# nanoporetech/bonito

Hardware: AMD Instinct MI355X
Metric: signal samples/sec/GPU (chunk=10000, batch=512) + read accuracy vs ref (higher is better)
Workload: dtype f16

## Files before the change

### bonito_amd/_lib.py

```python
import ctypes as C
import os

_HERE = os.path.dirname(os.path.abspath(__file__))
LIB_PATH = os.environ.get("BONITO_HIP_LIB") or os.path.join(_HERE, "libbonito_hip.so")


class HipEngineError(RuntimeError):
    """An entry point of libbonito_hip.so reported an error."""


class bh_layer_t(C.Structure):
    _fields_ = [
        ("kind", C.c_int32), ("in_size", C.c_int32), ("out_size", C.c_int32),
        ("winlen", C.c_int32), ("stride", C.c_int32), ("padding", C.c_int32),
        ("activation", C.c_int32), ("reverse", C.c_int32),
        ("nhead", C.c_int32), ("dim_ff", C.c_int32), ("win_left", C.c_int32), ("win_right", C.c_int32),
        ("scale_factor", C.c_int32), ("groups", C.c_int32), ("add_residual", C.c_int32), ("quantize", C.c_int32), ("reserved_i", C.c_int32 * 1),
        ("scale", C.c_float), ("clamp_lo", C.c_float), ("clamp_hi", C.c_float),
        ("blank_score", C.c_float), ("alpha", C.c_float), ("eps", C.c_float), ("reserved_f", C.c_float * 2),
        ("w0", C.c_void_p), ("b0", C.c_void_p), ("w1", C.c_void_p), ("b1", C.c_void_p),
        ("w2", C.c_void_p), ("w3", C.c_void_p), ("w4", C.c_void_p), ("w5", C.c_void_p),
    ]


BH_ACT = {None: 0, "none": 0, "swish": 1, "tanh": 2, "relu": 3}
BH_LAYER_CONV, BH_LAYER_LSTM, BH_LAYER_LINEAR_CRF, BH_LAYER_CLAMP = 1, 2, 3, 4
BH_LAYER_TRANSFORMER, BH_LAYER_UPSAMPLE, BH_LAYER_TCS_BLOCK, BH_LAYER_CTC_DECODER = 5, 6, 7, 8
BH_LAYER_DWCONV, BH_LAYER_RESIDUAL_PROJ, BH_LAYER_LINEAR = 9, 10, 11

_vp, _i, _f, _l, _sz = C.c_void_p, C.c_int, C.c_float, C.c_long, C.c_size_t

SIGNATURES = {
    "bh_last_error": (C.c_char_p, []),
    "bh_abi_version": (_i, []),
    "bh_sizeof_layer": (_sz, []),
    "bh_device_count": (_i, []),
    "bh_encoder_create": (_i, [C.POINTER(bh_layer_t), _i, _i, _i, _i, C.POINTER(_vp)]),
    "bh_encoder_destroy": (None, [_vp]),
    "bh_encoder_output_shape": (_i, [_vp, _i, C.POINTER(_i), C.POINTER(_i), C.POINTER(_i)]),
    "bh_encoder_forward": (_i, [_vp, _vp, _i, _i, _vp, _vp]),
    "bh_encoder_check": (_i, [_vp, _vp]),
    "bh_encoder_error_flag": (_i, [_vp]),
    "bh_encoder_last_ticket": (_l, [_vp]),
    "bh_encoder_error_flag_at": (_i, [_vp, _l]),
    "bh_encoder_ack": (_i, [_vp, _l]),
    "bh_encoder_describe": (_i, [_vp, C.c_char_p, _sz]),
    "bh_encoder_profile": (_i, [_vp, _i]),
    "bh_encoder_profile_read": (_i, [_vp, C.POINTER(C.c_float), C.POINTER(_i)]),
    "bh_crf_viterbi_workspace": (_sz, [_i, _i, _i]),
    "bh_crf_viterbi": (_i, [_vp, _i, _i, _i, _i, _f, _l, _l, _vp, _vp, _vp, _vp, _vp]),
    "bh_crf_reverse_complement": (_i, [_vp, _vp, _i, _i, _i, _i, _l, _l, _vp]),
    "bh_crf_logz": (_i, [_vp, _i, _i, _i, _f, _vp, _vp, _vp]),
    "bh_crf_seq_workspace": (_sz, [_i, _i, _i, _i]),
    "bh_crf_seq_logz": (_i, [_vp, _i, _i, _i, _i, _f, _l, _l, _vp, _i, _i, _vp, _vp, _vp, _vp]),
    "bh_crf_seq_viterbi": (_i, [_vp, _i, _i, _i, _i, _f, _l, _l, _vp, _i, _i, _vp, _vp, _vp, _vp, _vp]),
    "bh_crf_seq_logz_free": (_i, [_vp, _i, _i, _i, _f, _l, _l, _vp, _i, _i, _vp, _vp, _vp, _vp]),
    "bh_crf_logz_dense": (_i, [_vp, _i, _i, _i, _i, _f, _l, _l, _vp, _vp]),
    "bh_sw_workspace": (_sz, [_i, _i, _i]),
    "bh_sw_align": (_i, [_vp, _l, _vp, _vp, _l, _vp, _i, _i, _i, _i, _i, _vp, _sz, _vp, _vp, _l, _vp, _vp]),
    "bh_set_option": (_i, [C.c_char_p, _i]),
    "bh_signal_normalise": (_i, [_vp, _vp, _vp, _vp, _i, _i, C.c_double, C.c_double, C.c_double, C.c_double, C.c_double, C.c_double,
                            _i, _vp, _vp, _vp, _vp, _vp]),
    "bh_signal_chunks": (_i, [_vp, _vp, _vp, _vp, _vp, _vp, _vp, _vp, _vp, _vp, _i, _i, _vp, _vp]),
    "bh_crf_posterior_viterbi_workspace": (_sz, [_i, _i, _i]),
    "bh_crf_posterior_viterbi": (_i, [_vp, _i, _i, _i, _f, _vp, _vp, _vp, _vp]),
    "bh_beam_search_workspace": (_sz, [_i, _i, _i]),
    "bh_beam_search": (_i, [_vp, _i, _i, _i, _i, _f, _f, _f, _f, _vp, _vp, _vp, _vp, _vp, _vp]),
    "bh_linear": (_i, [_vp, _vp, _vp, _vp, _i, _i, _i, _i, _i, _i, _i, _f, _f, _f, _i, _i, _l, _l, _i, _vp]),
    "bh_linear_residual": (_i, [_vp, _vp, _vp, _vp, _i, _i, _i, _i, _i, _i, _i, _f, _f, _f, _i, _i, _l, _l, _i, _vp, _i, _f, _vp]),
    "bh_linear_qkv_rotary": (_i, [_vp, _vp, _vp, _vp, _i, _i, _i, _vp, _i, _f, _vp]),
    "bh_linear_last_kernel": (_i, []),
    "bh_conv1d_first": (_i, [_vp, _vp, _vp, _vp, _i, _i, _i, _i, _i, _i, _i, _f, _f, _l, _l, _vp]),
    "bh_conv1d_packed_halves": (_sz, [_i, _i, _i]),
    "bh_conv1d_pack": (_i, [_vp, _i, _i, _i, _vp]),
    "bh_conv1d": (_i, [_vp, _vp, _vp, _vp, _i, _i, _i, _i, _i, _i, _i, _i, _f, _f, _l, _l, _vp]),
    "bh_ctc_greedy_decode": (_i, [_vp, _vp, _i, _i, _f, _f, _vp, _vp, _vp, _vp, _vp]),
    "bh_ctc_beam_search_workspace": (_sz, [_l, _i, _i, _i]),
    "bh_ctc_beam_search": (_i, [_vp, _vp, _i, _i, _i, _f, _vp, _vp, _vp, _vp, _vp]),
    "bh_dwconv1d": (_i, [_vp, _vp, _vp, _i, _i, _i, _i, _i, _i, _vp]),
    "bh_rotary_table": (_i, [_i, _i, _vp]),
    "bh_attention": (_i, [_vp, _vp, _vp, _i, _i, _i, _i, _i, _i, _vp]),
    "bh_attention_prerotated": (_i, [_vp, _vp, _i, _i, _i, _i, _i, _i, _vp]),
    "bh_rmsnorm_residual": (_i, [_vp, _vp, _vp, _vp, _l, _i, _f, _f, _vp]),
    "bh_lstm_pack_whh": (_i, [_vp, _i, _vp]),
    "bh_host_compact": (_l, [_vp, _l, _vp]),
    "bh_host_chunk_rows": (_l, [_vp, _l, _i, _i, _l, _l, _vp]),
    "bh_host_format_read": (_l, [_vp, _vp, _vp, _vp, _i, _l, _l, _i, _i, _i, _i, _i, _i, C.c_double, C.c_char_p, C.c_char_p, _l, _l,
                                 _vp, _l, _vp, _vp]),
    "bh_host_mean_qscore": (C.c_double, [C.c_char_p, _l]),
    "bh_host_svb16_decode": (_l, [_vp, _l, _l, _vp]),
    "bh_lstm_workspace": (_sz, [_i, _i]),
    "bh_lstm_layer": (_i, [_vp, _vp, _vp, _i, _i, _i, _i, _vp, _vp, _i, _vp]),
    "bh_lstm_q8_layer": (_i, [_vp, _f, _vp, _vp, _vp, _i, _i, _i, _i, _i, _vp, _vp, _vp, _vp]),
    "bh_encoder_debug_read": (_i, [_vp, _vp, _sz, _sz]),
    "bh_encoder_set_option": (_i, [_vp, C.c_char_p, _i]),
}

_lib = None


def lib():
    global _lib
    if _lib is None:
        if not os.path.exists(LIB_PATH):
            raise HipEngineError(
                "%s not found: the MI355X engine is not built (run `python build.py`). "
                "bonito_amd has no CPU fallback." % LIB_PATH
            )
        import torch
        handle = C.CDLL(LIB_PATH)
        for name, (res, args) in SIGNATURES.items():
            fn = getattr(handle, name)
            fn.restype = res
            fn.argtypes = args
        if handle.bh_sizeof_layer() != C.sizeof(bh_layer_t):
            raise HipEngineError("bh_layer_t layout mismatch between include/bonito_hip.h and bonito_amd/_lib.py")
        _lib = handle
    return _lib


def last_error():
    msg = lib().bh_last_error()
    return msg.decode() if msg else ""


def check(rc, what=""):
    if rc != 0:
        raise HipEngineError("%s failed (rc=%d): %s" % (what or "libbonito_hip call", rc, last_error()))


def stream_ptr(device=None):
    import torch
    return C.c_void_p(torch.cuda.current_stream(device).cuda_stream)


def ptr(t):
    if t is None:
        return None
    return C.c_void_p(t.data_ptr())
```

### bonito_amd/csrc/abi.cpp

```cpp
#include <hip/hip_runtime.h>
#include <string.h>

#include <algorithm>
#include <cmath>
#include <vector>

#include "../../include/bonito_hip.h"
#include "common.h"
#include "devbuf.h"
#include "kernels.h"
#include "options.h"

extern "C" size_t bh_conv1d_packed_halves(int Cin, int Cout, int K) {
    size_t kp = ((size_t)K * Cin + 31) / 32 * 32;
    size_t c16 = ((size_t)Cout + 15) / 16 * 16;
    return kp * c16;
}
extern "C" int bh_conv1d_pack(const float* w, int Cin, int Cout, int K, uint16_t* packed) {
    BH_REQUIRE(w && packed && Cin > 0 && Cout > 0 && K > 0, "conv1d_pack: bad arguments");
    size_t kp = ((size_t)K * Cin + 31) / 32 * 32;
    size_t c16 = ((size_t)Cout + 15) / 16 * 16;
    memset(packed, 0, kp * c16 * 2);
    for (int f = 0; f < Cout; ++f)
        for (int c = 0; c < Cin; ++c)
// ... 25 lines not shown
                       row_s_hi, row_s_lo, row_lim, (hipStream_t)stream);
}
extern "C" int bh_linear_residual(const void* X, const void* W, const float* bias, void* out, int M, int N, int K, int ldx,
                                  int ldw, int ldo, int act, float scale, float clamp_lo, float clamp_hi, int gated,
                                  int row_div, long row_s_hi, long row_s_lo, int row_lim, const void* residual, int ldres,
                                  float res_scale, void* stream) {
    BH_REQUIRE(X && W && out && residual, "linear_residual: null pointer");
    return bh_k_linear(X, W, bias, out, M, N, K, ldx, ldw, ldo, act, scale, clamp_lo, clamp_hi, gated, row_div,
                       row_s_hi, row_s_lo, row_lim, (hipStream_t)stream, residual, ldres, res_scale);
}
extern "C" int bh_linear_qkv_rotary(const void* X, const void* W, const float* bias, void* out, int M, int D, int K,
                                    const float* cos_sin, int T, float qscale, void* stream) {
    BH_REQUIRE(X && W && out && cos_sin, "linear_qkv_rotary: null pointer");
    return bh_k_linear_qkv_rotary(X, W, bias, out, M, D, K, cos_sin, T, qscale, (hipStream_t)stream);
}
extern "C" int bh_linear_last_kernel(void) { return bh_k_linear_last_kernel(); }
extern "C" int bh_conv1d_first(const void* signal, const float* w, const float* bias, void* out, int N, int Lin,
                               int Cout, int K, int stride, int pad, int act, float clamp_lo, float clamp_hi,
                               long os_n, long os_t, void* stream) {
    BH_REQUIRE(signal && w && out && stride > 0, "conv1d_first: bad arguments");
    const int lout = conv_out_len(Lin, K, stride, pad);
    BH_REQUIRE(lout > 0, "conv1d_first: input too short");
    return bh_k_conv_first(signal, w, bias, out, N, Lin, lout, Cout, K, stride, pad, act, clamp_lo, clamp_hi, os_n,
                           os_t, (hipStream_t)stream);
}
extern "C" int bh_conv1d(const void* in, const void* wpacked, const float* bias, void* out, int N, int Lin, int Cin,
                         int Cout, int K, int stride, int pad, int act, float clamp_lo, float clamp_hi, long os_n,
                         long os_t, void* stream) {
    BH_REQUIRE(in && wpacked && out && stride > 0, "conv1d: bad arguments");
    const int lout = conv_out_len(Lin, K, stride, pad);
    BH_REQUIRE(lout > 0, "conv1d: input too short");
    return bh_k_conv_igemm(in, wpacked, bias, out, N, Lin, lout, Cin, Cout, K, stride, pad, act, clamp_lo, clamp_hi,
                           os_n, os_t, (hipStream_t)stream);
}
extern "C" int bh_rotary_table(int T, int dim, float* out) {
    BH_REQUIRE(out && T > 0 && dim > 0 && dim % 2 == 0, "rotary_table: bad arguments");
    const int half = dim / 2;
    for (int t = 0; t < T; ++t)
        for (int i = 0; i < half; ++i) {
            const float inv = 1.0f / powf(10000.0f, (float)(2 * i) / (float)dim);
            const float ang = (float)t * inv;
            out[((size_t)t * half + i) * 2] = cosf(ang);
            out[((size_t)t * half + i) * 2 + 1] = sinf(ang);
        }
    return 0;
}
extern "C" int bh_attention(const void* qkv, void* out, const float* cos_sin, int N, int T, int nhead, int head_dim,
                            int win_left, int win_right, void* stream) {
    BH_REQUIRE(qkv && out && cos_sin, "attention: null pointer");
    return bh_k_attention(qkv, out, cos_sin, N, T, nhead, head_dim, win_left, win_right, (hipStream_t)stream);
}
extern "C" int bh_attention_prerotated(const void* qkv, void* out, int N, int T, int nhead, int head_dim, int win_left, int win_right,
                                       void* stream) {
    BH_REQUIRE(qkv && out, "attention_prerotated: null pointer");
    return bh_k_attention_prerotated(qkv, out, N, T, nhead, head_dim, win_left, win_right, (hipStream_t)stream);
}
extern "C" int bh_rmsnorm_residual(const void* a, const void* x, const float* w, void* out, long M, int D, float alpha,
                                   float eps, void* stream) {
    BH_REQUIRE(a && x && w && out && M > 0, "rmsnorm_residual: bad arguments");
    return bh_k_rmsnorm_residual(a, x, w, out, M, D, alpha, eps, (hipStream_t)stream);
}
extern "C" int bh_ctc_greedy_decode(const float* logp, const long* offsets, int R, int classes, float qscale, float qbias,
                                    int8_t* labels, int8_t* qual, int* path, int* count, void* stream) {
    BH_REQUIRE(logp && offsets && labels && qual && path && count, "ctc_greedy_decode: null pointer");
    return bh_k_ctc_greedy(logp, offsets, R, classes, qscale, qbias, labels, qual, path, count, (hipStream_t)stream);
}
extern "C" size_t bh_ctc_beam_search_workspace(long total_steps, int R, int classes, int beam_size) {
    return bh_k_ctc_beam_workspace(total_steps, R, classes, beam_size);
}
extern "C" int bh_ctc_beam_search(const float* logp, const long* offsets, int R, int classes, int beam_size, float threshold,
                                  void* workspace, int8_t* labels, int* path, int* count, void* stream) {
    BH_REQUIRE(logp && offsets && workspace && labels && path && count, "ctc_beam_search: null pointer");
    return bh_k_ctc_prefix_beam(logp, offsets, R, classes, beam_size, threshold, workspace, labels, path, count,
                                (hipStream_t)stream);
}
extern "C" int bh_dwconv1d(const void* in, const float* w, void* out, int N, int Lin, int C, int K, int stride, int pad,
                           void* stream) {
    BH_REQUIRE(in && w && out && stride > 0, "dwconv1d: bad arguments");
    const int lout = conv_out_len(Lin, K, stride, pad);
    BH_REQUIRE(lout > 0, "dwconv1d: input too short");
    return bh_k_dwconv(in, w, out, N, Lin, lout, C, K, stride, pad, (hipStream_t)stream);
}
extern "C" size_t bh_lstm_workspace(int N, int H) { return bh_k_lstm_ws_bytes(N, H); }
extern "C" int bh_lstm_layer(const void* gates_in, const void* whh_packed, void* h_out, int T, int N, int H,
                             int reverse, void* workspace, int* err_flag, int flags, void* stream) {
    BH_REQUIRE(gates_in && whh_packed && h_out && err_flag && workspace, "lstm_layer: null pointer");
    BH_REQUIRE(T > 0, "lstm_layer: T must be positive");
    int rc = bh_k_fill_u16(h_out, 0xFFFFu, (size_t)T * N * H, (hipStream_t)stream);
    if (rc) return rc;
    if (H > 512 || (flags & 2)) {
        const int per = std::max(8, bh_k_lstm_geometry(BH_LSTM_STREAM, H).rings_per_launch(bh_cu_count()));
        for (int r0 = 0; r0 < N / 16; r0 += per) {
            const int nr = std::min(per, N / 16 - r0);
            rc = bh_k_lstm_layer_stream((const char*)gates_in + (size_t)r0 * 16 * 4 * H * 2, whh_packed,
                                        (char*)h_out + (size_t)r0 * 16 * H * 2, T, N, H, reverse, err_flag,
                                        (hipStream_t)stream, nr, (int*)workspace, flags & 1);
            if (rc) return rc;
        }
        return 0;
    }
    return bh_k_lstm_layer(gates_in, whh_packed, h_out, T, N, H, reverse, err_flag, (hipStream_t)stream, N / 16,
                           (int*)workspace, flags & 1);
}
extern "C" int bh_lstm_q8_layer(const void* x, float bound, const float* w_ih, const float* w_hh, const float* bias, int T, int N,
                                int H, int reverse, int variant, void* h16_out, int8_t* hq_frag, int32_t* sums, void* stream_) {
    BH_REQUIRE(x && w_ih && w_hh && h16_out && T > 0 && N > 0 && N % 16 == 0, "lstm_q8_layer: bad arguments");
    const int U = bh_k_lstm_q8_units(H, variant);
    BH_REQUIRE(U != 0, "lstm_q8_layer: hidden size %d is not covered by the 8-bit kernel", H);
    hipStream_t st = (hipStream_t)stream_;
    const int R = N / 16;
    const size_t tile = bh_k_lstm_q8_tile_bytes(H), wbytes = (size_t)4 * H * ((H + 63) / 64 * 64);
    std::vector<int8_t> pk(wbytes);
    std::vector<float> s_ih((size_t)4 * H), s_hh((size_t)4 * H), b((size_t)4 * H, 0.0f);
    DevBuf q_wih, q_whh, q_sx, q_sh, q_b, xq, ex, ws, err;
    if (bh_k_lstm_q8_pack(w_ih, H, U, pk.data(), s_ih.data()) || upload(q_wih, pk.data(), pk.size())) return -1;
    if (bh_k_lstm_q8_pack(w_hh, H, U, pk.data(), s_hh.data()) || upload(q_whh, pk.data(), pk.size())) return -1;
    const float xs = (float)((double)bound / 127.0);
    for (int j = 0; j < 4 * H; ++j) { s_ih[j] *= xs; s_hh[j] /= 127.0f; if (bias) b[j] = bias[j]; }
    if (upload_f32(q_sx, s_ih.data(), s_ih.size()) || upload_f32(q_sh, s_hh.data(), s_hh.size()) || upload_f32(q_b, b.data(), b.size())) return -1;
    if (xq.alloc((size_t)T * R * tile) || ex.alloc(4 * (size_t)R * tile) || ws.alloc(bh_k_lstm_ws_bytes(N, 1024)) || err.alloc(sizeof(int))) return -1;
    BH_CHECK_HIP(hipMemsetAsync(err.p, 0, sizeof(int), st));
    int rc = bh_k_quantise_rows(x, xq.p, T, N, H, R, bound, st);
    if (!rc) rc = bh_k_lstm_q8_arm(ex.p, R, H, st);
    if (rc) return rc;
    const int per = bh_k_lstm_q8_geometry(H, variant).rings_per_launch(bh_cu_count());
    BH_REQUIRE(per >= 1, "lstm_q8_layer: device has too few CUs for hidden size %d", H);
    for (int r0 = 0; r0 < R; r0 += per) {
        const int nr = std::min(per, R - r0);
        rc = bh_k_lstm_layer_q8((const char*)xq.p + (size_t)r0 * tile, q_wih.p, q_whh.p, (const float*)q_sx.p, (const float*)q_sh.p,
                                (const float*)q_b.p, hq_frag ? (char*)hq_frag + (size_t)r0 * tile : nullptr,
                                (char*)h16_out + (size_t)r0 * 16 * H * 2, (char*)ex.p + (size_t)r0 * tile, T, N, H, R, nr, reverse,
                                (int*)err.p, st, (int*)ws.p, 0, variant, sums ? sums + (size_t)r0 * 16 * 4 * H * 2 : nullptr,
                                (unsigned)bh::g_opt.lstm_max_spins);
        if (rc) return rc;
    }
    int flag = 0;
    BH_CHECK_HIP(hipMemcpyAsync(&flag, err.p, sizeof(int), hipMemcpyDeviceToHost, st));
    BH_CHECK_HIP(hipStreamSynchronize(st));
    BH_REQUIRE(flag == 0, "lstm_q8_layer: exchange timeout in the recurrent kernel");
    return 0;
}
extern "C" size_t bh_beam_search_workspace(int N, int T, int state_len) { return bh_k_beam_workspace(N, T, state_len); }
extern "C" int bh_beam_search(const void* scores, int N, int T, int state_len, int beam_width, float beam_cut,
                              float blank_score, float q_scale, float q_offset, void* workspace, int8_t* sequence,
                              int8_t* qstring, int8_t* moves, float* qfloat, void* stream) {
    BH_REQUIRE(scores && workspace && sequence && qstring && moves, "beam_search: null pointer");
    return bh_k_beam_search(scores, N, T, state_len, beam_width, beam_cut, blank_score, q_scale, q_offset, workspace,
                            sequence, qstring, moves, qfloat, (hipStream_t)stream);
}
extern "C" int bh_crf_reverse_complement(const void* in, void* out, int N, int T, int state_len, int layout_5s,
                                         long stride_n, long stride_t, void* stream) {
    BH_REQUIRE(in && out, "crf_reverse_complement: null pointer");
    return bh_k_crf_revcomp(in, out, N, T, state_len, layout_5s, stride_n, stride_t, (hipStream_t)stream);
}
extern "C" int bh_crf_logz(const void* scores, int N, int T, int state_len, float blank_score, void* workspace,
                           double* logz, void* stream) {
    BH_REQUIRE(scores && workspace && logz, "crf_logz: null pointer");
    return bh_k_crf_logz(scores, N, T, state_len, blank_score, workspace, logz, (hipStream_t)stream);
}
extern "C" size_t bh_crf_seq_workspace(int N, int T, int Lmax, int state_len) {
    return bh_k_crf_seq_workspace(N, T, Lmax, state_len);
}
extern "C" int bh_crf_seq_logz(const void* scores, int N, int T, int state_len, int layout_5s, float blank_score, long stride_n,
                               long stride_t, const void* targets, int Lmax, int target_bytes, const int32_t* target_lengths,
                               void* workspace, float* logz_out, void* stream) {
    BH_REQUIRE(scores && targets && target_lengths && workspace && logz_out, "crf_seq_logz: null pointer");
// ... 73 lines not shown
```

### bonito_amd/csrc/engine.cpp

```cpp
#include <hip/hip_runtime.h>
#include <stdarg.h>
#include <stdio.h>
#include <string.h>

#include <algorithm>
#include <atomic>
#include <cmath>
#include <string>
#include <vector>

#include "../../include/bonito_hip.h"
#include "common.h"
#include "devbuf.h"
#include "kernels.h"
#include "options.h"

static thread_local char g_err[1024] = "";
void bh_set_error(const char* fmt, ...) {
    va_list ap;
    va_start(ap, fmt);
    vsnprintf(g_err, sizeof(g_err), fmt, ap);
    va_end(ap);
}
extern "C" const char* bh_last_error(void) { return g_err; }
// ... 22 lines not shown
                    }
    return 0;
}

namespace {

struct Layer {
    bh_layer_t d;
    DevBuf w0, w1, w2, w3, w4, w5, b0, b1;
    bool fused_clamp = false;
    float clamp_lo = -INFINITY, clamp_hi = INFINITY;
    int cin_eff = 0, cout_eff = 0;
    bool pointwise = false;
    bool q8 = false;
    int q_variant = 0;
    float q_bound = 1.0f;
    DevBuf q_wih, q_whh, q_sx, q_sh;
};

enum Layout { L_SIGNAL, L_NLC, L_TNC };

struct ProfSpan {
    bh_encoder* e; hipStream_t st; int cls; hipEvent_t a = nullptr, b = nullptr;
    ProfSpan(bh_encoder* e_, hipStream_t st_, int cls_);
    ~ProfSpan();
};

static inline int pad8(int n) { return (n + 7) / 8 * 8; }

}

#include <mutex>
#include <unordered_map>
hipError_t bh_max_lds(const void* fn, int bytes) {
    static std::mutex mu;
    static std::unordered_map<unsigned long long, int> raised;
    int dev = 0;
    hipError_t e = hipGetDevice(&dev);
    if (e != hipSuccess) return e;
    const unsigned long long key = (unsigned long long)(uintptr_t)fn * 64ull + (unsigned)dev % 64u;
    {
        std::lock_guard<std::mutex> g(mu);
        auto it = raised.find(key);
        if (it != raised.end() && it->second >= bytes) return hipSuccess;
    }
    e = hipFuncSetAttribute(fn, hipFuncAttributeMaxDynamicSharedMemorySize, bytes);
    if (e == hipSuccess) {
        std::lock_guard<std::mutex> g(mu);
        int& have = raised[key];
        if (have < bytes) have = bytes;
    }
    return e;
}
int bh_cu_count() {
    static std::atomic<int> cached[64];
    int dev = 0, cus = 0;
    if (hipGetDevice(&dev) != hipSuccess || dev < 0 || dev >= 64) return 256;
    cus = cached[dev].load(std::memory_order_relaxed);
    if (cus > 0) return cus;
    if (hipDeviceGetAttribute(&cus, hipDeviceAttributeMultiprocessorCount, dev) != hipSuccess || cus <= 0) return 256;
    cached[dev].store(cus, std::memory_order_relaxed);
    return cus;
}

struct bh_encoder {
    int device = 0;
    int max_batch = 0, max_chunk = 0;
    int n_cus = 0;
    std::vector<Layer> layers;
    DevBuf act[3], gates, sig, err, lstm_ws;
    static constexpr int ERR_SLOTS = 64;
    int* err_host = nullptr;
    std::atomic<long> ticket{-1};
    std::atomic<long> checked{-1};
    std::atomic<int> sticky{0};
    int* cur_err = nullptr;
    int n_act = 2;
    hipStream_t fill_stream = nullptr;
    hipEvent_t fill_ready = nullptr, fill_done = nullptr;
    void* prefilled = nullptr;
    int lstm_prefill = 1;
    DevBuf q_act[2], q_ex;
    DevBuf ex16;
    int lstm_pair = 1;
    int norm_fuse = 0;
    int lstm_exchange = 1;
    int lstm_q8 = 1;
    DevBuf res;
    DevBuf t_qkv, t_mid, t_a, t_b, rot;
    int rot_len = 0;
    int out_features = 0;
    int lstm_force_slow = 0;
    int batch_pad = 16;
    int lstm_wide = 1;
    int attn_ring = 1;
    int lstm_fused = 3;
    bool profiling = false;
    struct Span { int cls; hipEvent_t a, b; };
    std::vector<Span> spans;
    ~bh_encoder() {
        for (auto& s : spans) { (void)hipEventDestroy(s.a); (void)hipEventDestroy(s.b); }
        if (fill_ready) (void)hipEventDestroy(fill_ready);
        if (fill_done) (void)hipEventDestroy(fill_done);
        if (fill_stream) (void)hipStreamDestroy(fill_stream);
        if (err_host) (void)hipHostFree(err_host);
    }
};

namespace {

ProfSpan::ProfSpan(bh_encoder* e_, hipStream_t st_, int cls_) : e(e_), st(st_), cls(cls_) {
    if (!e->profiling) return;
    if (hipEventCreate(&a) != hipSuccess || hipEventCreate(&b) != hipSuccess) { a = b = nullptr; return; }
    (void)hipEventRecord(a, st);
}
ProfSpan::~ProfSpan() {
    if (!a) return;
    (void)hipEventRecord(b, st);
    e->spans.push_back({cls, a, b});
}

struct Walk {
    int T = 0, C = 0;
    size_t act_bytes = 0, gate_bytes = 0;
    size_t qkv_bytes = 0, mid_bytes = 0, model_bytes = 0;
    int max_tokens = 0;
};
static int walk(const bh_encoder* e, int N, int L, Walk* w) {
    long len = L;
    int C = 1;
    size_t amax = 0;
    for (const auto& l : e->layers) {
        switch (l.d.kind) {
            case BH_LAYER_CONV:
                len = conv_out_len((int)len, l.d.winlen, l.d.stride, l.d.padding);
                BH_REQUIRE(len > 0, "encoder: chunk of %d samples is too short for the convolution stack", L);
                C = l.d.out_size;
                amax = std::max(amax, (size_t)N * len * std::max(l.cout_eff, C) * 2);
                break;
            case BH_LAYER_LSTM:
                C = l.d.out_size;
                amax = std::max(amax, (size_t)N * len * C * 2);
                w->gate_bytes = std::max(w->gate_bytes, (size_t)N * len * 4 * C * 2);
                break;
            case BH_LAYER_LINEAR_CRF:
                C = l.d.out_size;
                break;
            case BH_LAYER_LINEAR:
                C = l.d.out_size;
                amax = std::max(amax, (size_t)N * len * C * 2);
                break;
            case BH_LAYER_CLAMP:
                break;
            case BH_LAYER_TRANSFORMER: {
                const size_t M = (size_t)N * len;
                amax = std::max(amax, M * C * 2);
                w->qkv_bytes = std::max(w->qkv_bytes, M * 3 * l.d.in_size * 2);
                w->mid_bytes = std::max(w->mid_bytes, M * l.d.dim_ff * 2);
                w->model_bytes = std::max(w->model_bytes, M * l.d.in_size * 2);
                w->max_tokens = std::max(w->max_tokens, (int)len);
                break;
            }
            case BH_LAYER_DWCONV:
                len = conv_out_len((int)len, l.d.winlen, l.d.stride, l.d.padding);
                BH_REQUIRE(len > 0, "encoder: chunk of %d samples is too short for the convolution stack", L);
                amax = std::max(amax, (size_t)N * len * C * 2);
// ... 239 lines not shown
               "encoder_create: layer %zu: clamp must follow a convolution or linear layer", i);
    Layer& P = e->layers[i - 1];
    P.fused_clamp = true;
    P.clamp_lo = d.clamp_lo;
    P.clamp_hi = d.clamp_hi;
    cs.bound = std::max(fabsf(d.clamp_lo), fabsf(d.clamp_hi));
    return 0;
}

static int create_layer(bh_encoder* e, size_t i, const bh_layer_t& d, CreateState& cs) {
    Layer& L = e->layers[i];
    switch (d.kind) {
        case BH_LAYER_CONV: return create_conv(e, i, d, cs);
        case BH_LAYER_LSTM: return create_lstm(e, i, d, cs);
        case BH_LAYER_LINEAR_CRF:
            BH_REQUIRE(d.w0 && d.in_size > 0 && d.out_size > 0 && d.in_size % 8 == 0, "encoder_create: layer %zu: malformed linearcrfencoder", i);
            e->out_features = d.out_size;
            return create_linear(L, d, d.out_size);
        case BH_LAYER_LINEAR:
            BH_REQUIRE(d.w0 && d.in_size > 0 && d.out_size > 0 && d.in_size % 8 == 0 && d.out_size % 8 == 0 && cs.channels == d.in_size,
                       "encoder_create: layer %zu: linear needs in/out features %% 8 == 0 and %d input features (chain provides %d)", i,
                       d.in_size, cs.channels);
            cs.channels = cs.channels_eff = d.out_size;
            return create_linear(L, d, d.out_size);
        case BH_LAYER_TRANSFORMER: return create_transformer(e, i, d);
        case BH_LAYER_DWCONV:
            BH_REQUIRE(d.w0 && d.in_size > 0 && d.in_size % 8 == 0 && d.winlen > 0 && d.stride > 0 && cs.channels == d.in_size &&
                           cs.channels_eff == d.in_size,
                       "encoder_create: layer %zu: depthwise conv needs %d (multiple of 8) input channels, chain provides %d", i, d.in_size,
                       cs.channels);
            return upload_f32(L.w0, d.w0, (size_t)d.in_size * d.winlen);
        case BH_LAYER_RESIDUAL_PROJ:
            BH_REQUIRE(d.w0 && d.in_size % 8 == 0 && d.out_size % 8 == 0 && d.in_size > 0 && d.out_size > 0 && cs.channels == d.in_size &&
                           cs.channels_eff == d.in_size,
                       "encoder_create: layer %zu: residual projection shape mismatch", i);
            return create_with_bias(L, d, true);
        case BH_LAYER_CTC_DECODER:
            BH_REQUIRE(d.w0 && d.in_size % 8 == 0 && d.out_size >= 1 && d.out_size <= 8 && cs.channels == d.in_size,
                       "encoder_create: layer %zu: ctc decoder needs features %% 8 == 0 and <= 8 classes", i);
            e->out_features = d.out_size;
            return create_with_bias(L, d, false);
        case BH_LAYER_UPSAMPLE:
            BH_REQUIRE(d.w0 && d.in_size > 0 && d.scale_factor > 0 && d.in_size % 8 == 0, "encoder_create: layer %zu: malformed upsample", i);
            return create_linear(L, d, (size_t)d.scale_factor * d.in_size);
        case BH_LAYER_CLAMP: return create_clamp(e, i, d, cs);
        default: BH_REQUIRE(false, "encoder_create: layer %zu: kind %d is not supported by this build", i, d.kind);
    }
}

static int create_workspace(bh_encoder* e, const CreateState& cs) {
    const size_t n_layers = e->layers.size();
    const int last = e->layers[n_layers - 1].d.kind;
    BH_REQUIRE(last == BH_LAYER_LINEAR_CRF || last == BH_LAYER_CTC_DECODER ||
                   (n_layers >= 2 && last == BH_LAYER_CLAMP && e->layers[n_layers - 2].d.kind == BH_LAYER_LINEAR_CRF),
               "encoder_create: the chain must end in a linearcrfencoder (optionally followed by clamp) or a ctc decoder");
    const int Np = (e->max_batch + e->batch_pad - 1) / e->batch_pad * e->batch_pad;
    Walk w;
    if (walk(e, Np, e->max_chunk, &w)) return -2;
    const size_t ab = w.act_bytes;
    bool has_res = false;
    for (const auto& l : e->layers) has_res |= l.d.kind == BH_LAYER_RESIDUAL_PROJ;
    if (has_res && e->res.alloc(ab + 256)) return -1;
    for (size_t i = 0; i < n_layers; ++i)
        if (e->layers[i].d.kind == BH_LAYER_LSTM && next_kind(e, i) == BH_LAYER_LSTM) e->n_act = 3;
    if (e->n_act == 3) {
        if (e->act[2].alloc(ab + 256) || hipMemset(e->act[2].p, 0, e->act[2].bytes) != hipSuccess ||
            hipEventCreateWithFlags(&e->fill_ready, hipEventDisableTiming) != hipSuccess ||
            hipEventCreateWithFlags(&e->fill_done, hipEventDisableTiming) != hipSuccess) {
            bh_set_error("encoder_create: sentinel pre-fill resources");
            return -1;
        }
    }
    if (cs.any_q8) {
        if (e->q_act[0].alloc(ab + 256) || e->q_act[1].alloc(ab + 256) || e->q_ex.alloc((size_t)4 * (Np / 16) * 16 * 1024 + 256))
            return -1;
    }
    {
        size_t exb = 0;
        for (const auto& l : e->layers) {
            if (l.d.kind != BH_LAYER_LSTM) continue;
            if (lstm_may_share(l.d)) exb = std::max(exb, bh_k_lstm_wgx_ex_bytes(Np, l.d.out_size));
            if (lstm_may_wide(l.d)) exb = std::max(exb, bh_k_lstm_wide_ex_bytes(Np, l.d.out_size));
        }
        if (exb && e->ex16.alloc(exb + 256)) return -1;
    }
    if (e->act[0].alloc(ab + 256) || e->act[1].alloc(ab + 256) || e->gates.alloc(w.gate_bytes + 256) ||
        e->sig.alloc((size_t)Np * e->max_chunk * 2) || e->err.alloc(sizeof(int) * bh_encoder::ERR_SLOTS) ||
        e->lstm_ws.alloc(bh_k_lstm_ws_bytes(Np, 1024)))
        return -1;
    if (w.qkv_bytes) {
        if (e->t_qkv.alloc(w.qkv_bytes + 256) || e->t_mid.alloc(w.mid_bytes + 256) || e->t_a.alloc(w.model_bytes + 256) ||
            e->t_b.alloc(w.model_bytes + 256))
            return -1;
        std::vector<float> cs_table((size_t)w.max_tokens * 32 * 2);
        if (bh_rotary_table(w.max_tokens, 64, cs_table.data())) return -2;
        if (upload_f32(e->rot, cs_table.data(), cs_table.size())) return -1;
        e->rot_len = w.max_tokens;
    }
    if (hipHostMalloc((void**)&e->err_host, sizeof(int) * bh_encoder::ERR_SLOTS, hipHostMallocDefault) != hipSuccess) {
        bh_set_error("encoder_create: hipHostMalloc failed");
        return -1;
    }
    for (int i = 0; i < bh_encoder::ERR_SLOTS; ++i) e->err_host[i] = 0;
    e->cur_err = (int*)e->err.p;
    if (hipMemset(e->err.p, 0, sizeof(int) * bh_encoder::ERR_SLOTS) != hipSuccess || hipMemset(e->act[0].p, 0, e->act[0].bytes) != hipSuccess ||
        hipMemset(e->act[1].p, 0, e->act[1].bytes) != hipSuccess) {
        bh_set_error("encoder_create: hipMemset failed");
        return -1;
    }
    return 0;
}

}

extern "C" int bh_encoder_create(const bh_layer_t* layers, int n_layers, int device, int max_batch,
                                 int max_chunk, bh_encoder_t** out) {
    BH_REQUIRE(layers && n_layers > 0 && out, "encoder_create: bad arguments");
    BH_REQUIRE(max_batch > 0 && max_chunk > 0, "encoder_create: max_batch/max_chunk must be positive");
    int ndev = 0;
    BH_CHECK_HIP(hipGetDeviceCount(&ndev));
    BH_REQUIRE(ndev > 0, "encoder_create: no HIP device visible -- the MI355X engine has no CPU fallback");
    BH_REQUIRE(device >= 0 && device < ndev, "encoder_create: device %d out of range (%d visible)", device, ndev);
    int prev = 0;
    BH_CHECK_HIP(hipGetDevice(&prev));
    BH_CHECK_HIP(hipSetDevice(device));
    auto* e = new bh_encoder();
    e->device = device;
    e->max_batch = max_batch;
    e->max_chunk = max_chunk;
    auto fail = [&](int code) {
        delete e;
        (void)hipSetDevice(prev);
        return code;
    };
    if (hipDeviceGetAttribute(&e->n_cus, hipDeviceAttributeMultiprocessorCount, device) != hipSuccess) {
        bh_set_error("encoder_create: cannot query CU count");
        return fail(-1);
    }
    e->layers.resize(n_layers);
    for (int i = 0; i < n_layers; ++i) e->layers[i].d = layers[i];
    CreateState cs;
    for (int i = 0; i < n_layers; ++i) {
        if (int rc = create_layer(e, (size_t)i, layers[i], cs)) return fail(rc);
        bh_layer_t& d = e->layers[i].d;
        d.w0 = d.w1 = d.w2 = d.w3 = d.w4 = d.w5 = d.b0 = d.b1 = nullptr;
    }
    if (int rc = create_workspace(e, cs)) return fail(rc);
    (void)hipSetDevice(prev);
    *out = e;
    return 0;
}

extern "C" void bh_encoder_destroy(bh_encoder_t* enc) {
    if (!enc) return;
    int prev = 0;
    (void)hipGetDevice(&prev);
    (void)hipSetDevice(enc->device);
    delete enc;
    (void)hipSetDevice(prev);
}

extern "C" int bh_encoder_output_shape(const bh_encoder_t* enc, int L, int* T, int* C, int* stride) {
    BH_REQUIRE(enc && L > 0, "encoder_output_shape: bad arguments");
    Walk w;
    if (walk(enc, 16, L, &w)) return -2;
    if (T) *T = w.T;
    if (C) *C = w.C;
// ... 13 lines not shown
    const size_t ib = next_layer(e, i), ic = next_layer(e, ib);
    if (next_kind(e, i) != BH_LAYER_CONV || next_kind(e, ib) != BH_LAYER_CONV) return false;
    const Layer &a = e->layers[i], &b = e->layers[ib], &c = e->layers[ic];
    if (a.d.in_size != 1 || a.pointwise || b.pointwise || c.pointwise || b.d.add_residual || c.d.add_residual) return false;
    if (next_kind(e, ic) != BH_LAYER_LSTM) return false;
    if (!bh_k_conv_front3_ok(a.cout_eff, a.d.winlen, a.d.stride, b.cin_eff, b.cout_eff, b.d.winlen, b.d.stride, c.cin_eff, c.cout_eff,
                             c.d.winlen, c.d.stride))
        return false;
    if (a.d.out_size != b.d.in_size || b.d.out_size != c.d.in_size || c.cout_eff != c.d.out_size) return false;
    *j1 = ib;
    *j2 = ic;
    return true;
}
}

extern "C" int bh_encoder_describe(const bh_encoder_t* e, char* buf, size_t n) {
    BH_REQUIRE(e && buf && n > 0, "encoder_describe: bad arguments");
    std::string out;
    char line[256];
    int li = 0;
    for (const auto& l : e->layers) {
        const bh_layer_t& d = l.d;
        switch (d.kind) {
            case BH_LAYER_CONV: {
                size_t fj1 = 0, fj2 = 0;
                const bool front = d.in_size == 1 && conv_front3_at(e, (size_t)li, &fj1, &fj2);
                snprintf(line, sizeof(line), "%d conv %d->%d k%d s%d: %s\n", li, d.in_size, d.out_size, d.winlen, d.stride,
                         l.pointwise ? "gemm (pointwise)" : front ? "conv_front3_kernel (this and the next two convolutions in one kernel)"
                         : d.in_size == 1 ? "conv_first_kernel" : "conv_igemm_kernel / conv_ws_kernel");
                break;
            }
            case BH_LAYER_LSTM: {
                const LstmPlan p = lstm_plan(e, l, (e->max_batch + e->batch_pad - 1) / e->batch_pad * e->batch_pad);
                const int H = d.out_size, nks = H / 32, MT = bh_k_lstm_wg_units(H) / 4;
                char k[128];
                switch (p.family) {
                    case BH_LSTM_Q8: snprintf(k, sizeof(k), "lstm_layer_q8_kernel<%d,%d> (int8 W/x/h, i32 MFMA 16x16x64)", (H + 63) / 64, bh_k_lstm_q8_units(H, l.q_variant) / 4); break;
                    case BH_LSTM_CTA: snprintf(k, sizeof(k), "lstm_layer_cta_kernel<%d,%d>", nks, MT); break;
                    case BH_LSTM_WGX: snprintf(k, sizeof(k), "lstm_layer_%s_kernel<%d,%d>", p.pair_launch(p.n_rings) ? "wgx2" : "wgx", nks, MT); break;
                    case BH_LSTM_FUSED: snprintf(k, sizeof(k), "lstm_layer_fused_kernel<%d>", nks); break;
                    case BH_LSTM_WIDE: snprintf(k, sizeof(k), "gemm + lstm_layer_wide_kernel<%d,%s>", nks, p.handoff == HANDOFF_RING ? "true" : "false"); break;
                    case BH_LSTM_WAVE: snprintf(k, sizeof(k), "gemm + lstm_layer_kernel<%d,false>", nks); break;
                    default: snprintf(k, sizeof(k), "gemm + lstm_layer_kernel<%d,true> (weight streaming)", nks);
                }
                snprintf(line, sizeof(line), "%d lstm %d%s: %s\n", li, H, d.reverse ? " rev" : "", k);
                break;
            }
            case BH_LAYER_LINEAR_CRF: snprintf(line, sizeof(line), "%d linearcrfencoder %d->%d: gemm\n", li, d.in_size, d.out_size); break;
            case BH_LAYER_LINEAR: snprintf(line, sizeof(line), "%d linear %d->%d: gemm\n", li, d.in_size, d.out_size); break;
            case BH_LAYER_TRANSFORMER: {
                const bool ring = e->attn_ring && bh_k_attention_ring_serves(d.win_left, d.win_right);
                snprintf(line, sizeof(line), "%d transformer d%d h%d ff%d: gemm (Wqkv%s, out_proj, fc1 SwiGLU, fc2) + %s + rmsnorm_residual_kernel\n",
                         li, d.in_size, d.nhead, d.dim_ff, ring ? " + rotary" : "", ring ? "attention_ring_kernel" : "attention_kernel");
                break;
            }
            case BH_LAYER_UPSAMPLE: snprintf(line, sizeof(line), "%d linearupsample x%d: gemm\n", li, d.scale_factor); break;
            case BH_LAYER_CLAMP: snprintf(line, sizeof(line), "%d clamp: fused into the previous layer's epilogue\n", li); break;
            case BH_LAYER_DWCONV: snprintf(line, sizeof(line), "%d dwconv k%d: dwconv_kernel\n", li, d.winlen); break;
            case BH_LAYER_RESIDUAL_PROJ: snprintf(line, sizeof(line), "%d residual projection: gemm\n", li); break;
            case BH_LAYER_CTC_DECODER: snprintf(line, sizeof(line), "%d ctc decoder: ctc_head_kernel\n", li); break;
            default: snprintf(line, sizeof(line), "%d kind %d\n", li, d.kind);
        }
        out += line;
        ++li;
    }
    snprintf(buf, n, "%s", out.c_str());
    return 0;
}

namespace {

struct Cursor {
    const void* cur;
    Layout lay = L_SIGNAL;
    int len, C = 1;
    int which = 0;
    const void* cur_q = nullptr;
    int qi = 0;
    bool res_ready = false;
    int N, Np;
    hipStream_t st;
    void* scores;
    int n_act;
    void advance(void* dst) { cur = dst; which = (which + 1) % n_act; }
};

static int prefill_next(bh_encoder* e, const Cursor& c, size_t i, size_t rows) {
    if (e->n_act != 3 || !e->lstm_prefill || e->profiling) return 0;
    const size_t j = next_layer(e, i);
    if (j >= e->layers.size() || e->layers[j].d.kind != BH_LAYER_LSTM) return 0;
    const Layer& nx = e->layers[j];
    if (lstm_plan(e, nx, c.Np).handoff != HANDOFF_OUTPUT) return 0;
    if (!e->fill_stream) BH_CHECK_HIP(hipStreamCreateWithFlags(&e->fill_stream, hipStreamNonBlocking));
    void* spare = e->act[(c.which + 1) % 3].p;
    BH_CHECK_HIP(hipEventRecord(e->fill_ready, c.st));
    BH_CHECK_HIP(hipStreamWaitEvent(e->fill_stream, e->fill_ready, 0));
    const int rc = bh_k_fill_u16(spare, 0xFFFFu, rows * nx.d.out_size, e->fill_stream);
    if (rc) return rc;
    BH_CHECK_HIP(hipEventRecord(e->fill_done, e->fill_stream));
    e->prefilled = spare;
    return 0;
}

static int forward_conv(bh_encoder* e, size_t& i, Cursor& c) {
    const Layer& l = e->layers[i];
    const bh_layer_t& d = l.d;
    hipStream_t st = c.st;
    const int Np = c.Np, len = c.len;
    BH_REQUIRE(c.lay == L_SIGNAL || c.lay == L_NLC, "encoder_forward: convolution after a time-major layer");
    BH_REQUIRE(c.C == d.in_size, "encoder_forward: layer %zu expects %d channels, got %d", i, d.in_size, c.C);
    size_t fj1 = 0, fj2 = 0;
    if (c.lay == L_SIGNAL && conv_front3_at(e, i, &fj1, &fj2)) {
        const Layer &l2 = e->layers[fj1], &l3 = e->layers[fj2];
        const int len1 = conv_out_len(len, d.winlen, d.stride, d.padding);
        const int len2 = conv_out_len(len1, l2.d.winlen, l2.d.stride, l2.d.padding);
        const int len3 = conv_out_len(len2, l3.d.winlen, l3.d.stride, l3.d.padding);
        BH_REQUIRE(len1 > 0 && len2 > 0 && len3 > 0, "encoder_forward: chunk too short for the convolution stack");
        void* dst3 = e->act[c.which].p;
        int rc3 = prefill_next(e, c, fj2, (size_t)len3 * Np);
        if (rc3) return rc3;
        ProfSpan span(e, st, BH_PROF_CONV);
        rc3 = bh_k_conv_front3(c.cur, Np, len, (const float*)l.w0.p, (const float*)l.b0.p, d.winlen, d.padding, d.activation, l.clamp_lo,
                               l.clamp_hi, l2.w0.p, (const float*)l2.b0.p, l2.d.winlen, l2.d.padding, l2.d.activation, l2.clamp_lo,
                               l2.clamp_hi, l3.w0.p, (const float*)l3.b0.p, l3.cout_eff, l3.d.winlen, l3.d.stride, l3.d.padding,
                               l3.d.activation, l3.clamp_lo, l3.clamp_hi, dst3, (long)l3.cout_eff, (long)Np * l3.cout_eff, st);
        if (rc3) return rc3;
        c.advance(dst3); c.len = len3; c.C = l3.d.out_size; c.lay = L_TNC;
        i = fj2;
        return 0;
    }
    const int lout = conv_out_len(len, d.winlen, d.stride, d.padding);
    void* dst = e->act[c.which].p;
    const bool tnc = next_kind(e, i) == BH_LAYER_LSTM;
    const int co = l.cout_eff;
    const long os_n = tnc ? co : (long)lout * co;
    const long os_t = tnc ? (long)Np * co : co;
    int rc;
    if (tnc) { rc = prefill_next(e, c, i, (size_t)lout * Np); if (rc) return rc; }
    ProfSpan span(e, st, BH_PROF_CONV);
    if (l.pointwise && !tnc) {
        const void* rsd = d.add_residual ? e->res.p : nullptr;
        BH_REQUIRE(!d.add_residual || c.res_ready, "encoder_forward: layer %zu adds a residual that was never projected", i);
        rc = bh_k_linear(c.cur, l.w0.p, (const float*)l.b0.p, dst, Np * len, d.out_size, d.in_size, d.in_size,
                         d.in_size, d.out_size, d.activation, 1.0f, l.clamp_lo, l.clamp_hi, 0, 0, 0, 0, 0, st, rsd, d.out_size);
        if (d.add_residual) c.res_ready = false;
    } else if (c.lay == L_SIGNAL)
        rc = bh_k_conv_first(c.cur, (const float*)l.w0.p, (const float*)l.b0.p, dst, Np, len, lout,
                             co, d.winlen, d.stride, d.padding, d.activation, l.clamp_lo, l.clamp_hi, os_n, os_t, st);
    else
        rc = bh_k_conv_igemm(c.cur, l.w0.p, (const float*)l.b0.p, dst, Np, len, lout, l.cin_eff,
                             co, d.winlen, d.stride, d.padding, d.activation, l.clamp_lo, l.clamp_hi, os_n, os_t, st);
    if (rc) return rc;
    c.advance(dst); c.len = lout; c.C = d.out_size; c.lay = tnc ? L_TNC : L_NLC;
    return 0;
}

static int forward_lstm_q8(bh_encoder* e, size_t i, Cursor& c, const LstmPlan& p) {
    const Layer& l = e->layers[i];
    const bh_layer_t& d = l.d;
    hipStream_t st = c.st;
    const int H = d.out_size, len = c.len, Np = c.Np, R = p.n_rings;
    const size_t tile = bh_k_lstm_q8_tile_bytes(H);
    void* dst = e->act[c.which].p;
    const size_t j = next_layer(e, i);
    const bool next_q8 = j < e->layers.size() && e->layers[j].d.kind == BH_LAYER_LSTM && lstm_plan(e, e->layers[j], Np).family == BH_LSTM_Q8;
    int rc;
    const void* xq = c.cur_q;
    if (!xq) {
        ProfSpan span(e, st, BH_PROF_OTHER);
        rc = bh_k_quantise_rows(c.cur, e->q_act[c.qi].p, len, Np, H, R, l.q_bound, st);
        if (rc) return rc;
        xq = e->q_act[c.qi].p;
        c.qi ^= 1;
    }
    void* hq_out = next_q8 ? e->q_act[c.qi].p : nullptr;
    void* h16_out = next_q8 ? nullptr : dst;
    ProfSpan span(e, st, BH_PROF_LSTM_REC);
    rc = bh_k_lstm_q8_arm(e->q_ex.p, R, H, st);
    if (rc) return rc;
    for (int r0 = 0; r0 < R; r0 += p.rings_per_launch) {
        const int nr = std::min(p.rings_per_launch, R - r0);
        rc = bh_k_lstm_layer_q8((const char*)xq + (size_t)r0 * tile, l.q_wih.p, l.q_whh.p, (const float*)l.q_sx.p,
                                (const float*)l.q_sh.p, (const float*)l.b0.p,
                                hq_out ? (char*)hq_out + (size_t)r0 * tile : nullptr,
                                h16_out ? (char*)h16_out + (size_t)r0 * 16 * H * 2 : nullptr,
                                (char*)e->q_ex.p + (size_t)r0 * tile, len, Np, H, R, nr, d.reverse, e->cur_err, st,
                                (int*)e->lstm_ws.p, e->lstm_force_slow, l.q_variant, nullptr, (unsigned)bh::g_opt.lstm_max_spins);
        if (rc) return rc;
    }
    if (next_q8) { c.cur_q = hq_out; c.qi ^= 1; }
    else { c.cur_q = nullptr; c.advance(dst); }
    c.C = H;
    return 0;
}

static int forward_lstm(bh_encoder* e, size_t i, Cursor& c) {
    const Layer& l = e->layers[i];
    const bh_layer_t& d = l.d;
    hipStream_t st = c.st;
    BH_REQUIRE(c.lay == L_TNC, "encoder_forward: lstm needs time-major input");
    BH_REQUIRE(c.C == d.in_size, "encoder_forward: layer %zu expects %d features, got %d", i, d.in_size, c.C);
    const int H = d.out_size, len = c.len, Np = c.Np;
    const int M = len * Np;
    const LstmPlan p = lstm_plan(e, l, Np);
    BH_REQUIRE(p.rings_per_launch >= 1, "encoder_forward: device has too few CUs (%d) for hidden size %d", e->n_cus, H);
    if (p.family == BH_LSTM_Q8) return forward_lstm_q8(e, i, c, p);
    BH_REQUIRE(c.cur_q == nullptr, "encoder_forward: layer %zu would read int8 activations it cannot consume", i);
    int rc;
    void* dst = e->act[c.which].p;
    if (p.gate_w) {
        ProfSpan span(e, st, BH_PROF_LSTM_GEMM);
        rc = bh_k_linear(c.cur, p.gate_w, p.gate_b, e->gates.p, M, 4 * H, d.in_size, d.in_size, d.in_size, 4 * H, bh::ACT_NONE, 1.0f,
                         -INFINITY, INFINITY, 0, 0, 0, 0, 0, st);
        if (rc) return rc;
    }
    if (p.handoff == HANDOFF_OUTPUT) {
        if (e->prefilled == dst) {
            BH_CHECK_HIP(hipStreamWaitEvent(st, e->fill_done, 0));
        } else {
            ProfSpan span(e, st, BH_PROF_FILL);
            rc = bh_k_fill_u16(dst, 0xFFFFu, (size_t)M * H, st);
            if (rc) return rc;
        }
    }
    e->prefilled = nullptr;
    if (next_kind(e, i) == BH_LAYER_LSTM) { rc = prefill_next(e, c, i, (size_t)M); if (rc) return rc; }
    ProfSpan span(e, st, BH_PROF_LSTM_REC);
    const int n_rings = p.n_rings, rev = d.reverse, slow = e->lstm_force_slow;
    int* ws = (int*)e->lstm_ws.p;
    const float* bias = (const float*)l.b0.p;
    for (int r0 = 0; r0 < n_rings;) {
        const bool pair = p.pair_launch(n_rings - r0);
        const int nr = std::min(pair ? 2 * p.rings_per_launch : p.rings_per_launch, n_rings - r0);
        const size_t col = (size_t)r0 * p.geo.ring_chunks;
        const char* x = (const char*)c.cur + col * H * 2;
        const char* g = (const char*)e->gates.p + col * 4 * H * 2;
        char* h = (char*)dst + col * H * 2;
        char* ex = e->ex16.p ? (char*)e->ex16.p + (size_t)r0 * (p.geo.ring_chunks / 16) * (H / 32) * 1024 : nullptr;
        switch (pair ? BH_LSTM_WGX2 : p.family) {
            case BH_LSTM_WGX2:
                rc = bh_k_lstm_layer_wgx2(x, l.w4.p, bias, l.w3.p, h, ex, len, Np, H, n_rings, rev, e->cur_err, st, nr, ws, slow, r0 == 0);
                break;
            case BH_LSTM_WGX:
                rc = bh_k_lstm_layer_wgx(x, l.w4.p, bias, l.w3.p, h, ex, len, Np, H, n_rings, rev, e->cur_err, st, nr, ws, slow, r0 == 0);
                break;
            case BH_LSTM_WIDE:
                rc = bh_k_lstm_layer_wide(g, l.w3.p, h, len, Np, H, rev, e->cur_err, st, nr, ws, slow,
                                          p.handoff == HANDOFF_RING ? ex : nullptr, n_rings, r0 == 0);
                break;
            case BH_LSTM_CTA: rc = bh_k_lstm_layer_cta(x, l.w4.p, bias, l.w3.p, h, len, Np, H, rev, st, nr); break;
            case BH_LSTM_FUSED: rc = bh_k_lstm_layer_fused(x, l.w2.p, bias, l.w1.p, h, len, Np, H, rev, e->cur_err, st, nr, ws, slow); break;
            case BH_LSTM_WAVE: rc = bh_k_lstm_layer(g, l.w1.p, h, len, Np, H, rev, e->cur_err, st, nr, ws, slow); break;
            default: rc = bh_k_lstm_layer_stream(g, l.w1.p, h, len, Np, H, rev, e->cur_err, st, nr, ws, slow);
        }
        if (rc) return rc;
        r0 += nr;
    }
    c.advance(dst); c.C = H;
    return 0;
}

static int forward_linear_crf(bh_encoder* e, size_t i, Cursor& c) {
    const Layer& l = e->layers[i];
    const bh_layer_t& d = l.d;
    BH_REQUIRE(c.lay == L_TNC || c.lay == L_NLC, "encoder_forward: linearcrfencoder needs encoded input");
    BH_REQUIRE(c.C == d.in_size, "encoder_forward: layer %zu expects %d features, got %d", i, d.in_size, c.C);
    const float sc = d.scale != 0.0f ? d.scale : 1.0f;
    int rc;
    ProfSpan span(e, c.st, BH_PROF_CRF_LINEAR);
    if (c.lay == L_TNC)
        rc = bh_k_linear(c.cur, l.w0.p, (const float*)l.b0.p, c.scores, c.len * c.Np, d.out_size, d.in_size, d.in_size,
                         d.in_size, d.out_size, d.activation, sc, l.clamp_lo, l.clamp_hi, 0, c.Np, 1, c.len, c.N, c.st);
    else
        rc = bh_k_linear(c.cur, l.w0.p, (const float*)l.b0.p, c.scores, c.len * c.N, d.out_size, d.in_size, d.in_size,
                         d.in_size, d.out_size, d.activation, sc, l.clamp_lo, l.clamp_hi, 0, 0, 0, 0, 0, c.st);
    if (rc) return rc;
    c.C = d.out_size;
    return 0;
}

static int forward_linear(bh_encoder* e, size_t i, Cursor& c) {
    const Layer& l = e->layers[i];
    const bh_layer_t& d = l.d;
    BH_REQUIRE(c.lay == L_TNC || c.lay == L_NLC, "encoder_forward: linear needs encoded input");
    BH_REQUIRE(c.C == d.in_size, "encoder_forward: layer %zu expects %d features, got %d", i, d.in_size, c.C);
    void* dst = e->act[c.which].p;
    ProfSpan span(e, c.st, BH_PROF_OTHER);
    int rc = bh_k_linear(c.cur, l.w0.p, (const float*)l.b0.p, dst, c.len * c.Np, d.out_size, d.in_size, d.in_size, d.in_size,
                         d.out_size, bh::ACT_NONE, 1.0f, l.clamp_lo, l.clamp_hi, 0, 0, 0, 0, 0, c.st);
    if (rc) return rc;
    c.advance(dst); c.C = d.out_size;
    return 0;
}

static int forward_transformer(bh_encoder* e, size_t i, Cursor& c) {
    const Layer& l = e->layers[i];
    const bh_layer_t& d = l.d;
    hipStream_t st = c.st;
    const int len = c.len, N = c.N;
    BH_REQUIRE(c.lay == L_NLC, "encoder_forward: transformer layer needs [N][T][D] input");
    BH_REQUIRE(c.C == d.in_size, "encoder_forward: layer %zu expects d_model %d, got %d", i, d.in_size, c.C);
    BH_REQUIRE(len <= e->rot_len, "encoder_forward: %d tokens exceed the rotary table (%d)", len, e->rot_len);
    const int D = d.in_size, F = d.dim_ff;
    const int M = N * len;
    const float eps = d.eps > 0.0f ? d.eps : 1e-5f;
    int rc;
    const bool ring = e->attn_ring && bh_k_attention_ring_serves(d.win_left, d.win_right);
    const bool fuse = e->norm_fuse != 0;
    auto proj_norm = [&](const void* x, const void* w, const float* b, int K, const void* res, const float* gain, void* y) {
        int r = bh_k_linear(x, w, b, e->t_b.p, M, D, K, K, K, D, bh::ACT_NONE, 1.0f, -INFINITY, INFINITY, 0, 0, 0, 0, 0, st,
                            fuse ? res : nullptr, fuse ? D : 0, fuse ? d.alpha : 1.0f);
        if (!r) r = bh_k_rmsnorm_residual(e->t_b.p, fuse ? nullptr : res, gain, y, M, D, d.alpha, eps, st);
        return r;
    };
    {
        ProfSpan span(e, st, BH_PROF_ATTENTION);
        if (ring)
            rc = bh_k_linear_qkv_rotary(c.cur, l.w0.p, (const float*)l.b0.p, e->t_qkv.p, M, D, D, (const float*)e->rot.p,
                                        len, 0.125f * 1.4426950408889634f, st);
        else
            rc = bh_k_linear(c.cur, l.w0.p, (const float*)l.b0.p, e->t_qkv.p, M, 3 * D, D, D, D, 3 * D, bh::ACT_NONE,
                             1.0f, -INFINITY, INFINITY, 0, 0, 0, 0, 0, st);
        if (rc) return rc;
    }
    {
        ProfSpan span(e, st, BH_PROF_ATTENTION_CORE);
        if (ring)
            rc = bh_k_attention_prerotated(e->t_qkv.p, e->t_a.p, N, len, d.nhead, D / d.nhead, d.win_left, d.win_right, st);
        else
            rc = bh_k_attention(e->t_qkv.p, e->t_a.p, (const float*)e->rot.p, N, len, d.nhead, D / d.nhead,
                                d.win_left, d.win_right, st);
// ... 20 lines not shown
    return 0;
}

static int forward_dwconv(bh_encoder* e, size_t i, Cursor& c) {
    const Layer& l = e->layers[i];
    const bh_layer_t& d = l.d;
    BH_REQUIRE(c.lay == L_NLC && c.C == d.in_size, "encoder_forward: depthwise conv needs [N][L][%d] input", d.in_size);
    const int lout = conv_out_len(c.len, d.winlen, d.stride, d.padding);
    void* dst = e->act[c.which].p;
    ProfSpan span(e, c.st, BH_PROF_CONV);
    int rc = bh_k_dwconv(c.cur, (const float*)l.w0.p, dst, c.Np, c.len, lout, c.C, d.winlen, d.stride, d.padding, c.st);
    if (rc) return rc;
    c.advance(dst); c.len = lout;
    return 0;
}

static int forward_residual_proj(bh_encoder* e, size_t i, Cursor& c) {
    const Layer& l = e->layers[i];
    const bh_layer_t& d = l.d;
    BH_REQUIRE(c.lay == L_NLC && c.C == d.in_size, "encoder_forward: residual projection needs [N][L][%d] input", d.in_size);
    ProfSpan span(e, c.st, BH_PROF_CONV);
    int rc = bh_k_linear(c.cur, l.w0.p, (const float*)l.b0.p, e->res.p, c.Np * c.len, d.out_size, d.in_size, d.in_size,
                         d.in_size, d.out_size, bh::ACT_NONE, 1.0f, -INFINITY, INFINITY, 0, 0, 0, 0, 0, c.st);
    if (rc) return rc;
    c.res_ready = true;
    return 0;
}

static int forward_ctc_decoder(bh_encoder* e, size_t i, Cursor& c) {
    const Layer& l = e->layers[i];
    const bh_layer_t& d = l.d;
    BH_REQUIRE(c.lay == L_NLC && c.C == d.in_size, "encoder_forward: ctc decoder needs [N][T][%d] input", d.in_size);
    ProfSpan span(e, c.st, BH_PROF_CRF_LINEAR);
    int rc = bh_k_ctc_head(c.cur, (const float*)l.w0.p, (const float*)l.b0.p, c.scores, (long)c.N * c.len, d.in_size, d.out_size, c.st);
    if (rc) return rc;
    c.C = d.out_size;
    return 0;
}

static int forward_upsample(bh_encoder* e, size_t i, Cursor& c) {
    const Layer& l = e->layers[i];
    const bh_layer_t& d = l.d;
    BH_REQUIRE(c.lay == L_NLC && c.C == d.in_size, "encoder_forward: upsample needs [N][T][%d] input", d.in_size);
    const int D = d.in_size, sf = d.scale_factor;
    void* dst = e->act[c.which].p;
    ProfSpan span(e, c.st, BH_PROF_OTHER);
    int rc = bh_k_linear(c.cur, l.w0.p, (const float*)l.b0.p, dst, c.N * c.len, sf * D, D, D, D, sf * D, bh::ACT_NONE,
                         1.0f, -INFINITY, INFINITY, 0, 0, 0, 0, 0, c.st);
    if (rc) return rc;
    c.advance(dst); c.len *= sf;
    return 0;
}

}

extern "C" int bh_encoder_forward(bh_encoder_t* e, const void* signal, int N, int L, void* scores, void* stream_) {
    BH_REQUIRE(e && signal && scores, "encoder_forward: null argument");
    BH_REQUIRE(N > 0 && N <= e->max_batch, "encoder_forward: batch %d outside 1..%d", N, e->max_batch);
    BH_REQUIRE(L > 0 && L <= e->max_chunk, "encoder_forward: chunk %d outside 1..%d", L, e->max_chunk);
    hipStream_t st = (hipStream_t)stream_;
    int prev = 0;
    BH_CHECK_HIP(hipGetDevice(&prev));
    if (prev != e->device) BH_CHECK_HIP(hipSetDevice(e->device));
    struct Restore {
        int prev, dev;
        ~Restore() { if (prev != dev) (void)hipSetDevice(prev); }
    } restore{prev, e->device};

    {
        const long n = ++e->ticket;
        const int slot = (int)(n % bh_encoder::ERR_SLOTS);
        if (n - bh_encoder::ERR_SLOTS > e->checked.load()) e->sticky.fetch_or(((volatile int*)e->err_host)[slot]);
        ((volatile int*)e->err_host)[slot] = 0;
        e->cur_err = (int*)e->err.p + slot;
        BH_CHECK_HIP(hipMemsetAsync(e->cur_err, 0, sizeof(int), st));
    }
    const int Np = (N + e->batch_pad - 1) / e->batch_pad * e->batch_pad;
    if (Np != N) BH_CHECK_HIP(hipMemsetAsync((char*)e->sig.p + (size_t)N * L * 2, 0, (size_t)(Np - N) * L * 2, st));
    BH_CHECK_HIP(hipMemcpyAsync(e->sig.p, signal, (size_t)N * L * 2, hipMemcpyDeviceToDevice, st));

    e->prefilled = nullptr;
    Cursor c;
    c.cur = e->sig.p; c.len = L; c.N = N; c.Np = Np; c.st = st; c.scores = scores; c.n_act = e->n_act;
    for (size_t i = 0; i < e->layers.size(); ++i) {
        int rc = 0;
        switch (e->layers[i].d.kind) {
            case BH_LAYER_CLAMP: continue;
            case BH_LAYER_CONV: rc = forward_conv(e, i, c); break;
            case BH_LAYER_LSTM: rc = forward_lstm(e, i, c); break;
            case BH_LAYER_LINEAR_CRF: rc = forward_linear_crf(e, i, c); break;
            case BH_LAYER_LINEAR: rc = forward_linear(e, i, c); break;
            case BH_LAYER_TRANSFORMER: rc = forward_transformer(e, i, c); break;
            case BH_LAYER_DWCONV: rc = forward_dwconv(e, i, c); break;
            case BH_LAYER_RESIDUAL_PROJ: rc = forward_residual_proj(e, i, c); break;
            case BH_LAYER_CTC_DECODER: rc = forward_ctc_decoder(e, i, c); break;
            case BH_LAYER_UPSAMPLE: rc = forward_upsample(e, i, c); break;
            default: BH_REQUIRE(false, "encoder_forward: unsupported layer kind %d", e->layers[i].d.kind);
        }
        if (rc) return rc;
    }
    BH_CHECK_HIP(hipMemcpyAsync(e->err_host + (e->cur_err - (int*)e->err.p), e->cur_err, sizeof(int), hipMemcpyDeviceToHost, st));
    return 0;
}

extern "C" long bh_encoder_last_ticket(const bh_encoder_t* e) { return e ? e->ticket.load() : -1; }

extern "C" int bh_encoder_error_flag_at(const bh_encoder_t* e, long ticket) {
    if (!e || !e->err_host) return 0;
    const long cur = e->ticket.load();
    if (ticket < 0 || ticket > cur) return 0;
    if (cur - ticket >= bh_encoder::ERR_SLOTS) {
        bh_set_error("forward %ld is more than %d forwards old: its timeout flag has been recycled", ticket, bh_encoder::ERR_SLOTS);
        return -1;
    }
    const int flag = ((volatile const int*)e->err_host)[ticket % bh_encoder::ERR_SLOTS];
    if (flag) bh_set_error("device-side timeout in a persistent kernel (flag=%d, forward %ld): the scores of that forward are invalid", flag, ticket);
    return flag;
}

extern "C" int bh_encoder_ack(bh_encoder_t* e, long ticket) {
    BH_REQUIRE(e && e->err_host, "encoder_ack: null engine");
    const long cur = e->ticket.load();
    BH_REQUIRE(ticket >= 0 && ticket <= cur, "encoder_ack: forward %ld has not been issued (last %ld)", ticket, cur);
    if (cur - ticket >= bh_encoder::ERR_SLOTS) {
        bh_set_error("forward %ld is more than %d forwards old: its timeout flag has been recycled", ticket, bh_encoder::ERR_SLOTS);
        return -1;
    }
    ((volatile int*)e->err_host)[ticket % bh_encoder::ERR_SLOTS] = 0;
    return 0;
}

static int pending_flags(const bh_encoder_t* e) {
    int flag = e->sticky.load();
    const long cur = e->ticket.load();
    long lo = e->checked.load() + 1;
    if (lo < cur - bh_encoder::ERR_SLOTS + 1) lo = cur - bh_encoder::ERR_SLOTS + 1;
    if (lo < 0) lo = 0;
    for (long n = lo; n <= cur; ++n) flag |= ((volatile const int*)e->err_host)[n % bh_encoder::ERR_SLOTS];
    return flag;
}

extern "C" int bh_encoder_error_flag(const bh_encoder_t* e) {
    if (!e || !e->err_host) return 0;
    const int flag = pending_flags(e);
    if (flag) bh_set_error("device-side timeout in a persistent kernel (flag=%d): the scores of that forward are invalid", flag);
    return flag;
}

extern "C" int bh_encoder_check(bh_encoder_t* e, void* stream_) {
    BH_REQUIRE(e, "encoder_check: null engine");
    BH_CHECK_HIP(hipStreamSynchronize((hipStream_t)stream_));
    const int flag = pending_flags(e);
    e->sticky.store(0);
    if (flag) bh_set_error("device-side timeout in a persistent kernel (flag=%d)", flag);
    e->checked.store(e->ticket.load());
    return flag;
}

extern "C" int bh_encoder_profile(bh_encoder_t* e, int enable) {
    BH_REQUIRE(e, "encoder_profile: null engine");
    e->profiling = enable != 0;
    return 0;
}
extern "C" int bh_encoder_profile_read(bh_encoder_t* e, float* ms, int* launches) {
    BH_REQUIRE(e && ms && launches, "encoder_profile_read: null argument");
    for (int i = 0; i < BH_PROF_CLASSES; ++i) { ms[i] = 0.0f; launches[i] = 0; }
    for (auto& s : e->spans) {
        BH_CHECK_HIP(hipEventSynchronize(s.b));
        float t = 0.0f;
        BH_CHECK_HIP(hipEventElapsedTime(&t, s.a, s.b));
        if (s.cls >= 0 && s.cls < BH_PROF_CLASSES) { ms[s.cls] += t; launches[s.cls] += 1; }
        (void)hipEventDestroy(s.a); (void)hipEventDestroy(s.b);
    }
    e->spans.clear();
    return 0;
}

extern "C" int bh_encoder_debug_read(bh_encoder_t* e, void* host, size_t bytes, size_t offset) {
    BH_REQUIRE(e && host && offset + bytes <= e->lstm_ws.bytes, "encoder_debug_read: out of range");
    BH_CHECK_HIP(hipMemcpy(host, (char*)e->lstm_ws.p + offset, bytes, hipMemcpyDeviceToHost));
    return 0;
}
extern "C" int bh_encoder_set_option(bh_encoder_t* e, const char* name, int value) {
    BH_REQUIRE(e && name, "encoder_set_option: null argument");
    if (!strcmp(name, "lstm_force_slow")) { e->lstm_force_slow = (e->lstm_force_slow & ~1) | (value & 1); return 0; }
    if (!strcmp(name, "lstm_fused")) { e->lstm_fused = value; return 0; }
    if (!strcmp(name, "attn_ring")) { e->attn_ring = value; return 0; }
    if (!strcmp(name, "lstm_wide")) { e->lstm_wide = value; return 0; }
    if (!strcmp(name, "lstm_prefill")) { e->lstm_prefill = value; return 0; }
    if (!strcmp(name, "lstm_q8")) { e->lstm_q8 = value; return 0; }
    if (!strcmp(name, "lstm_exchange")) { e->lstm_exchange = value; return 0; }
    if (!strcmp(name, "lstm_pair")) { e->lstm_pair = value; return 0; }
    if (!strcmp(name, "norm_fuse")) { e->norm_fuse = value; return 0; }
    if (!strcmp(name, "gemm_v1")) { bh::g_opt.gemm_path = value; return 0; }
    if (!strcmp(name, "lstm_tune")) { e->lstm_force_slow = (e->lstm_force_slow & 1) | (value << 8); return 0; }
    BH_REQUIRE(false, "encoder_set_option: unknown option '%s'", name);
}
```

### bonito_amd/csrc/kernels.h

```cpp
#pragma once
#include <hip/hip_runtime.h>
#include <stdint.h>

int bh_k_linear(const void* X, const void* W, const float* bias, void* out, int M, int N, int K,
                int ldx, int ldw, int ldo, int act, float scale, float clamp_lo, float clamp_hi,
                int gated, int row_div, long row_s_hi, long row_s_lo, int row_lim, hipStream_t stream,
                const void* residual = nullptr, int ldres = 0, float res_scale = 1.0f);
int bh_k_linear_last_kernel();

int bh_k_conv_first(const void* signal, const float* w, const float* bias, void* out, int N, int Lin,
                    int Lout, int Cout, int K, int stride, int pad, int act, float clamp_lo,
                    float clamp_hi, long os_n, long os_t, hipStream_t stream);
int bh_k_conv_igemm(const void* in, const void* wpk, const float* bias, void* out, int N, int Lin,
                    int Lout, int Cin, int Cout, int K, int stride, int pad, int act, float clamp_lo,
                    float clamp_hi, long os_n, long os_t, hipStream_t stream);

enum bh_lstm_family { BH_LSTM_WAVE, BH_LSTM_FUSED, BH_LSTM_STREAM, BH_LSTM_WGX, BH_LSTM_WGX2, BH_LSTM_CTA, BH_LSTM_WIDE, BH_LSTM_Q8 };
struct bh_lstm_geometry {
    int ring_chunks = 16;
    int wgs_per_group = 0;
    int rings_per_slot = 1;
    int wgs_per_cu = 1;
    bool unlimited = false;
    int grid(int n_rings) const {
// ... 20 lines not shown
size_t bh_k_lstm_packed_bytes(int H);
int bh_k_lstm_wg_units(int H);
int bh_k_lstm_cta_units(int H);
int bh_k_lstm_layer_cta(const void* x, const void* wih_tiles, const float* bias, const void* whh_tiles, void* h_out, int T, int N,
                        int H, int reverse, hipStream_t stream, int n_rings);

int bh_k_crf_viterbi(const void* scores, int N, int T, int state_len, int layout_5s, float blank_score,
                     long s_n, long s_t, void* bp_ws, float* alpha_ws, int8_t* moves, int8_t* path,
                     float* best_score, hipStream_t stream);

int bh_k_crf_revcomp(const void* in, void* out, int N, int T, int state_len, int layout_5s, long s_n, long s_t,
                     hipStream_t stream);

size_t bh_k_crf_seq_workspace(int N, int T, int Lmax, int state_len);
int bh_k_crf_seq(const void* scores, int N, int T, int state_len, int layout_5s, float blank, long s_n, long s_t,
                 const void* targets, int target_bytes, int Lmax, const int* lens, void* workspace, float* out, int* align,
                 int mode, hipStream_t stream);
int bh_k_crf_logz_dense(const void* scores, int N, int T, int state_len, int layout_5s, float blank, long s_n, long s_t,
                        float* out, hipStream_t stream);

size_t bh_k_sw_workspace(int n, int max_seq, int max_ref);
int bh_k_sw_align(const void* seqs, long seq_stride, const int* seq_lens, const void* refs, long ref_stride, const int* ref_lens,
                  int n, int match, int mismatch, int gap_open, int gap_extend, void* workspace, size_t workspace_bytes,
                  int* result, unsigned* ops, long ops_stride, int* n_ops, hipStream_t stream);

size_t bh_k_beam_workspace(int N, int T, int state_len);
int bh_k_crf_logz(const void* scores, int N, int T, int state_len, float blank, void* workspace, double* logz_out,
                   hipStream_t stream);
int bh_k_beam_search(const void* scores, int N, int T, int state_len, int beam_width, float beam_cut,
                     float blank, float q_scale, float q_offset, void* workspace, int8_t* sequence,
                     int8_t* qstring, int8_t* moves, float* qfloat, hipStream_t stream);

int bh_k_attention(const void* qkv, void* out, const float* cos_sin, int N, int T, int nhead, int head_dim,
                   int win_left, int win_right, hipStream_t stream);
int bh_k_rmsnorm_residual(const void* a, const void* x, const float* w, void* out, long M, int D, float alpha,
                          float eps, hipStream_t stream);

int bh_k_dwconv(const void* in, const float* w, void* out, int N, int Lin, int Lout, int C, int K, int stride,
                int pad, hipStream_t stream);
int bh_k_ctc_head(const void* in, const float* w, const float* bias, void* out, long M, int features, int classes,
                  hipStream_t stream);
int bh_k_ctc_greedy(const float* logp, const long* offs, int R, int C, float qscale, float qbias, int8_t* seq,
                    int8_t* qual, int* path, int* count, hipStream_t stream);
size_t bh_k_ctc_beam_workspace(long total_steps, int R, int C, int beam_size);
int bh_k_ctc_prefix_beam(const float* logp, const long* offs, int R, int C, int beam_size, float threshold, void* workspace,
                         int8_t* labels, int* path, int* count, hipStream_t stream);
size_t bh_k_posterior_viterbi_workspace(int N, int T, int state_len);
int bh_k_posterior_viterbi(const void* scores, int N, int T, int state_len, float blank, void* workspace, int8_t* moves,
                           int8_t* path, hipStream_t stream);
int bh_k_conv_front3_ok(int c1_eff, int K1, int s1, int c2_in_eff, int c2_eff, int K2, int s2, int c3_in_eff, int c3_out, int K3, int s3);
int bh_k_conv_front3(const void* signal, int N, int L0, const float* w1, const float* b1, int K1, int pad1, int act1, float lo1, float hi1,
                     const void* w2pk, const float* b2, int K2, int pad2, int act2, float lo2, float hi2, const void* w3pk,
                     const float* b3, int Cout3, int K3, int stride3, int pad3, int act3, float lo3, float hi3, void* out, long os_n,
                     long os_t, hipStream_t stream);
int bh_k_linear_qkv_rotary(const void* X, const void* W, const float* bias, void* out, int M, int D, int K, const float* cos_sin,
                           int T, float qscale, hipStream_t stream);
int bh_k_attention_prerotated(const void* qkv, void* out, int N, int T, int nhead, int head_dim, int win_left, int win_right,
                              hipStream_t stream);
inline bool bh_k_attention_ring_serves(int win_left, int win_right) {
    return win_left >= 0 && win_right >= 0 && win_left <= 128 && win_right <= 144;
}
int bh_k_signal_normalise(const int16_t* raw, const long* offs, const float* cal_scale, const float* cal_offset, int R,
                          int strategy, double qa, double qb, double shift_mult, double scale_mult, double fixed_shift,
                          double fixed_scale, int do_trim, double* shift, double* scale, int* weak, int* trim, hipStream_t stream);
int bh_k_signal_chunks(const int16_t* raw, const long* offs, const float* cal_scale, const float* cal_offset, const double* shift,
                       const double* scale, const int* weak, const int* chunk_read, const long* chunk_start, const long* chunk_len,
                       int n_chunks, int L, void* out, hipStream_t stream);
int bh_k_lstm_wide_ok(int H);
int bh_k_lstm_layer_wide(const void* gates_perm, const void* whh_tiles, void* h_out, int T, int N, int H, int reverse,
                         int* err_flag, hipStream_t stream, int n_rings, int* xcc_ws, int force_slow, void* ex = nullptr, int R = 0,
                         int arm = 0);
size_t bh_k_lstm_wide_ex_bytes(int N, int H);

int bh_k_lstm_q8_units(int H, int variant);
bh_lstm_geometry bh_k_lstm_q8_geometry(int H, int variant);
size_t bh_k_lstm_q8_tile_bytes(int H);
int bh_k_lstm_q8_pack(const float* w, int H, int U, int8_t* packed, float* scale);
int bh_k_quantise_rows(const void* x, void* out, int T, int N, int H, int R, float bound, hipStream_t stream);
int bh_k_lstm_q8_arm(void* ex, int R, int H, hipStream_t stream);
int bh_k_lstm_layer_q8(const void* xq, const void* wih, const void* whh, const float* sx, const float* sh, const float* bias,
                       void* hq_out, void* h16_out, void* ex, int T, int N, int H, int R, int n_rings, int reverse, int* err_flag,
                       hipStream_t stream, int* xcc_ws, int flags, int variant, int* dbg, unsigned max_spins);
size_t bh_k_lstm_wgx_ex_bytes(int N, int H);
int bh_k_lstm_layer_wgx(const void* x, const void* wih_tiles, const float* bias, const void* whh_tiles, void* h_out, void* ex, int T,
                        int N, int H, int R, int reverse, int* err_flag, hipStream_t stream, int n_rings, int* xcc_ws, int force_slow,
                        int arm);
int bh_k_lstm_layer_wgx2(const void* x, const void* wih_tiles, const float* bias, const void* whh_tiles, void* h_out, void* ex, int T,
                        int N, int H, int R, int reverse, int* err_flag, hipStream_t stream, int n_rings, int* xcc_ws, int force_slow,
                        int arm);
```

### bonito_amd/csrc/lstm.hip

```cpp
#include <string.h>
#include <type_traits>

#include "common.h"
#include "kernels.h"
#include "options.h"

namespace bh {

struct LstmArgs {
    const half_t* G;
    const half_t* whh;
    half_t* h;
    int T, N, H;
    int n_rings;
    int reverse;
    int* err;
    unsigned max_spins;
    int* xcc_ws;
    int force_slow;
    int tune;
};

__device__ __forceinline__ int xcc_id() {
    return (int)(__builtin_amdgcn_s_getreg(20 | (0 << 6) | (3 << 11)) & 0xF);
}

__device__ __forceinline__ bool ring_store_policy(const LstmArgs& p, int ring, int slice, int nsl, int lane) {
    int* slot = p.xcc_ws + (long)ring * nsl;
    const int mine = xcc_id();
    if (lane == 0) __hip_atomic_store(slot + slice, mine, __ATOMIC_RELAXED, __HIP_MEMORY_SCOPE_AGENT);
    unsigned spins = 0;
    bool ok = false;
    while (true) {
        bool any_unset = false, any_other = false;
        for (int i = lane; i < nsl; i += 64) {
            const int v = __hip_atomic_load(slot + i, __ATOMIC_RELAXED, __HIP_MEMORY_SCOPE_AGENT);
            any_unset |= v < 0;
            any_other |= v != mine;
        }
        if (!__any(any_unset)) { ok = !__any(any_other); break; }
        if (++spins > p.max_spins) break;
        __builtin_amdgcn_s_sleep(4);
    }
    return ok && !p.force_slow;
}

constexpr unsigned SENTINEL_MASK = 0x40004000u;

typedef unsigned short __attribute__((may_alias)) u16_alias_t;
typedef unsigned long long __attribute__((may_alias)) u64_alias_t;

__device__ __forceinline__ float tanh_gate(float x) { return __builtin_fmaf(-2.0f, rcpf_(__expf(2.0f * x) + 1.0f), 1.0f); }

__device__ __forceinline__ float lstm_cell(float ai, float af, float ag, float ao, float& c) {
    const float ei = __expf(-__builtin_amdgcn_fmed3f(ai, -25.0f, 25.0f));
    const float ef = __expf(-__builtin_amdgcn_fmed3f(af, -25.0f, 25.0f));
    const float eg = __expf(-2.0f * __builtin_amdgcn_fmed3f(ag, -12.5f, 12.5f));
    const float eo = __expf(-__builtin_amdgcn_fmed3f(ao, -25.0f, 25.0f));
    const float didg = __fmul_rn(1.0f + ei, 1.0f + eg);
    const float df = 1.0f + ef;
    const float num = __builtin_fmaf(c, didg, __fmul_rn(1.0f - eg, df));
    c = __fmul_rn(num, rcpf_(__fmul_rn(df, didg)));
    const float ec = __expf(-2.0f * __builtin_amdgcn_fmed3f(c, -12.5f, 12.5f));
    const float hv = __fmul_rn(1.0f - ec, rcpf_(__fmul_rn(1.0f + ec, 1.0f + eo)));
    return (fabsf(hv) <= 1.0f) ? hv : 0.0f;
}

template <int NKS, bool STREAM>
__global__ __launch_bounds__(256, 1) void lstm_layer_kernel(LstmArgs p) {
    const int lane = threadIdx.x & 63;
    const int wave = __builtin_amdgcn_readfirstlane(threadIdx.x >> 6);
    constexpr int H = NKS * 32;
    constexpr int NSL = H / 16;
    const int xcd = blockIdx.x & 7;
    const int lwg = blockIdx.x >> 3;
    constexpr int WPR = NSL / 4;
    const int rg = STREAM ? lwg / WPR : lwg / NSL;
    const int slice = STREAM ? (lwg - rg * WPR) * 4 + wave : lwg - rg * NSL;
    const int ring = STREAM ? rg * 8 + xcd : (rg * 4 + wave) * 8 + xcd;
    if (ring >= p.n_rings) return;
    const half_t* wbase = p.whh + ((long)slice * 4 * NKS * 64 + lane) * 8;

    half8_t w[STREAM ? 1 : 4][STREAM ? 1 : NKS];
// ... 248 lines not shown
        }
        half4_t ho;
#pragma unroll
        for (int i = 0; i < 4; ++i) {
            const float hv = lstm_cell(acc[0][i], acc[1][i], acc[2][i], acc[3][i], cst[i]);
            ho[i] = (half_t)hv;
        }
#pragma unroll
        for (int ks = 0; ks < NKS; ++ks) asm volatile("" : "+v"(xf[ks]));
        unsigned long long packed = __builtin_bit_cast(unsigned long long, ho);
        unsigned long long* dst = (unsigned long long*)(p.h + ((long)t * p.N + n) * H + hu0);
        if (fast) *dst = packed;
        else __hip_atomic_store(dst, packed, __ATOMIC_RELAXED, __HIP_MEMORY_SCOPE_AGENT);
        if (p.tune & 4) st_rec += __builtin_readcyclecounter() - pc3;
    }
    if ((p.tune & 4) && lane == 0) {
        long long* st = (long long*)((char*)p.xcc_ws + (((size_t)p.n_rings * NSL * sizeof(int) + 64 + 7) & ~(size_t)7)) + ((long)ring * NSL + slice) * 8;
        st[0] = __builtin_readcyclecounter() - st_t0;
        st[1] = st_poll;
        st[2] = st_rounds;
        st[3] = st_first_ok;
        st[4] = st_x;
        st[5] = st_re;
        st[6] = st_rec;
        st[7] = st_hist;
    }
}

__device__ __forceinline__ void mfma16_av(const half8_t& a_agpr, const half8_t& b, float4_t& c) {
    asm("v_mfma_f32_16x16x32_f16 %0, %1, %2, %0" : "+v"(c) : "a"(a_agpr), "v"(b));
}
__device__ __forceinline__ void mfma16_vv(const half8_t& a, const half8_t& b, float4_t& c) {
    asm("v_mfma_f32_16x16x32_f16 %0, %1, %2, %0" : "+v"(c) : "v"(a), "v"(b));
}
template <int MT>
__device__ __forceinline__ void mfma_settle_v(float4_t (&c)[MT]) {
    if constexpr (MT == 3) asm volatile("s_nop 15\n\ts_nop 7" : "+v"(c[0]), "+v"(c[1]), "+v"(c[2]));
    else asm volatile("s_nop 15\n\ts_nop 7" : "+v"(c[0]), "+v"(c[1]), "+v"(c[2]), "+v"(c[3]));
}

__device__ __forceinline__ unsigned lds_addr(const char* p) { return (unsigned)(size_t)(__attribute__((address_space(3))) const char*)p; }
#include "ringstep3_mfma.inc"
#include "ringstep3p_mfma.inc"
template <int NKS, int MT>
__device__ __forceinline__ void ring_stream(float4_t (&xacc)[MT], float (&cst)[MT], float (&hv)[MT], const half8_t (&whh)[MT][NKS],
                                            const half8_t (&wih)[MT][NKS], const float4_t (&bias)[MT], unsigned hb, unsigned xb) {
    if constexpr (NKS == 12 && MT == 3) ringstep3_mfma(xacc, cst, hv, whh, wih, bias, hb, xb);
}
template <int NKS, int MT, int KQ>
__device__ __forceinline__ void ring_stream_paired(float4_t (&xacc)[MT], float (&cst)[MT], float (&hv)[MT], const half8_t (&whh)[MT][NKS],
                                                   const half8_t (&wih)[MT][NKS], const float4_t (&bias)[MT], unsigned hb, unsigned xb,
                                                   unsigned long long& bad, unsigned pm0, const char* exo, const unsigned (&vp)[KQ],
                                                   unsigned xm0, const char* xsrc, unsigned vx, unsigned hbo, unsigned sga, unsigned rda,
                                                   unsigned vmy, unsigned vh, const char* exs, const char* exa, const char* hrow, unsigned fast) {
    if constexpr (NKS == 12 && MT == 3)
        ringstep3p_mfma(xacc, cst, hv, whh, wih, bias, hb, xb, bad, pm0, exo, vp, xm0, xsrc, vx, hbo, sga, rda, vmy, vh, exs, exa, hrow, fast);
}
#include "ringstep3u_mfma.inc"
template <int NKS, int MT, int KQ, int HOFF, int XOFF, int VOFF, int PMO, int XMO>
__device__ __forceinline__ void ring_stream_unrolled(float4_t (&xacc)[MT], float (&cst)[MT], float (&hv)[MT], const half8_t (&whh)[MT][NKS],
                                                     const half8_t (&wih)[MT][NKS], const float4_t (&bias)[MT], unsigned hb, unsigned xb,
                                                     unsigned long long& bad, unsigned pm0, const char* exo, const unsigned (&vp)[KQ],
                                                     unsigned xm0, const char* xsrc, unsigned vx, unsigned hbo, unsigned sga, unsigned rda,
                                                     unsigned vmy, unsigned vh, const char* exs, const char* exa, const char* hrow, unsigned fast) {
    if constexpr (NKS == 12 && MT == 3)
        ringstep3u_mfma<HOFF, XOFF, VOFF, PMO, XMO>(xacc, cst, hv, whh, wih, bias, hb, xb, bad, pm0, exo, vp, xm0, xsrc, vx, hbo, sga, rda, vmy, vh, exs,
                                                    exa, hrow, fast);
}
#include "ringstep3r_mfma.inc"
template <int NKS, int MT>
__device__ __forceinline__ void ring_stream_rec(float4_t (&xacc)[MT], float (&cst)[MT], float (&hv)[MT], const half8_t (&whh)[MT][NKS],
                                                const half8_t (&wih)[MT][NKS], const float4_t (&bias)[MT], unsigned hb) {
    if constexpr (NKS == 12 && MT == 3) ringstep3r_mfma(xacc, cst, hv, whh, wih, bias, hb, 0u);
}
__device__ __forceinline__ void dma16_wgx(const char* g, char* lds) {
    const unsigned l = (unsigned)__builtin_amdgcn_readfirstlane((int)(unsigned)(size_t)(__attribute__((address_space(3))) char*)lds);
    asm volatile("s_mov_b32 m0, %0\n\ts_nop 0\n\tglobal_load_lds_dwordx4 %1, off" ::"s"(l), "v"(g) : "memory");
}

struct LstmWgxArgs {
    LstmFusedArgs f;
    char* ex;
    int R;
};

template <int IMM, bool POLL>
__device__ __forceinline__ void dma16_s(const char* sbase, unsigned voff, unsigned lds_a) {
    if constexpr (POLL)
        asm volatile("s_mov_b32 m0, %0\n\ts_nop 0\n\tglobal_load_lds_dwordx4 %1, %2 offset:%3 sc0 sc1" ::"s"(lds_a), "v"(voff), "s"(sbase), "i"(IMM) : "memory");
    else
        asm volatile("s_mov_b32 m0, %0\n\ts_nop 0\n\tglobal_load_lds_dwordx4 %1, %2 offset:%3" ::"s"(lds_a), "v"(voff), "s"(sbase), "i"(IMM) : "memory");
}
template <bool SC1>
__device__ __forceinline__ void store8_s(const char* sbase, unsigned voff, unsigned long long v) {
    if constexpr (SC1) asm volatile("global_store_dwordx2 %0, %1, %2 sc1" ::"v"(voff), "v"(v), "s"(sbase) : "memory");
    else asm volatile("global_store_dwordx2 %0, %1, %2" ::"v"(voff), "v"(v), "s"(sbase) : "memory");
}

template <int NKS, int MT>
__global__ __launch_bounds__(256, 1) void lstm_layer_wgx_kernel(LstmWgxArgs wp) {
    extern __shared__ __attribute__((aligned(16))) char smem[];
    const LstmFusedArgs& fp = wp.f;
    const LstmArgs& p = fp.a;
    constexpr int H = NKS * 32, U = 4 * MT, NSL = H / U, WPR = NSL / 4, KQ = (NKS + 3) / 4, TILE = NKS * 1024;
    constexpr bool EXACT = NKS % 4 == 0;
    static_assert(H % (4 * U) == 0, "four slices per workgroup");
    const int lane = threadIdx.x & 63;
    const int wave = __builtin_amdgcn_readfirstlane(threadIdx.x >> 6);
    const int xcd = blockIdx.x & 7;
    const int lwg = blockIdx.x >> 3;
    const int rl = lwg / WPR;
    const int ring = rl * 8 + ((p.tune & 32) ? ((xcd + (lwg - rl * WPR)) & 7) : xcd);
    const int slice = (lwg - rl * WPR) * 4 + wave;
    if (ring >= p.n_rings) return;

    char* hbuf = smem;
    char* xbuf = smem + 2 * TILE;
    char* stage = smem + 5 * TILE + wave * (16 * U * 2);

    half8_t whh[MT][NKS], wih[MT][NKS];
#pragma unroll
    for (int m = 0; m < MT; ++m)
#pragma unroll
        for (int ks = 0; ks < NKS; ++ks) {
            const long o = ((((long)slice * MT + m) * NKS + ks) * 64 + lane) * 8;
            whh[m][ks] = *(const half8_t*)(p.whh + o);
            wih[m][ks] = *(const half8_t*)(fp.wih + o);
        }
    const int c = lane & 15, q = lane >> 4;
    float cst[MT];
    float4_t bias4[MT];
#pragma unroll
    for (int m = 0; m < MT; ++m) {
        cst[m] = 0.f;
#pragma unroll
        for (int i = 0; i < 4; ++i) bias4[m][i] = fp.bias[i * H + slice * U + q * MT + m];
    }
    bool dead = false;
    const bool fast = ring_store_policy(p, ring, slice, NSL, lane);

    int t = p.reverse ? p.T - 1 : 0;
    const int dt = p.reverse ? -1 : 1;
    const half_t* xptr = fp.x + ((long)(ring * 16 + c) * H + q * 8);
    const long x_row = (long)p.N * H;
    const int lo = lane * 16;
    const long slot_stride = (long)wp.R * TILE;
    char* exr = wp.ex + (long)ring * TILE;

    constexpr int PARTS = U / 4;
    const bool mover = lane < 16 * PARTS;
    const int cc = lane / PARTS, part = lane - cc * PARTS;
    const int u0 = slice * U + part * 4;
    const int my_byte = (((u0 >> 5) * 64 + ((u0 >> 3) & 3) * 16 + cc) << 4) + (u0 & 7) * 2;

    uint4_t hq[KQ];
    float4_t xacc[MT];
    auto x_phase = [&](const char* xb) {
#pragma unroll
        for (int m = 0; m < MT; ++m) xacc[m] = bias4[m];
        half8_t b_cur = *(const half8_t*)(xb + lo), b_nxt = b_cur;
#pragma unroll
        for (int ks = 0; ks < NKS; ++ks) {
            if (ks + 1 < NKS) b_nxt = *(const half8_t*)(xb + (ks + 1) * 1024 + lo);
#pragma unroll
            for (int m = 0; m < MT; ++m) {
                if (m < MT - 1) mfma16_av(wih[m][ks], b_cur, xacc[m]);
                else mfma16_vv(wih[m][ks], b_cur, xacc[m]);
// ... 122 lines not shown
            u16_alias_t* sg = (u16_alias_t*)stage + c * U + q * MT;
#pragma unroll
            for (int m = 0; m < MT; ++m) sg[m] = __builtin_bit_cast(unsigned short, ho[m]);
            if (mover) {
                const unsigned long long packed = *(const u64_alias_t*)((half_t*)stage + cc * U + part * 4);
                if constexpr (STREAM) {
                    const char* exs = exr + (long)(step & 3) * slot_stride;
                    if (fast) store8_s<false>(exs, (unsigned)my_byte, packed); else store8_s<true>(exs, (unsigned)my_byte, packed);
                    if (step >= 2 && step + 2 < p.T) {
                        const char* exa = exr + (long)((step + 2) & 3) * slot_stride;
                        if (fast) store8_s<false>(exa, (unsigned)my_byte, ~0ull); else store8_s<true>(exa, (unsigned)my_byte, ~0ull);
                    }
                    store8_s<false>((const char*)p.h + (long)t * row_bytes, vh_off, packed);
                } else {
                unsigned long long* dst = (unsigned long long*)(exr + (long)(step & 3) * slot_stride + my_byte);
                if (fast) *dst = packed;
                else __hip_atomic_store(dst, packed, __ATOMIC_RELAXED, __HIP_MEMORY_SCOPE_AGENT);
                if (step >= 2 && step + 2 < p.T) {
                    unsigned long long* ra = (unsigned long long*)(exr + (long)((step + 2) & 3) * slot_stride + my_byte);
                    if (fast) *ra = ~0ull;
                    else __hip_atomic_store(ra, ~0ull, __ATOMIC_RELAXED, __HIP_MEMORY_SCOPE_AGENT);
                }
                *(unsigned long long*)(p.h + ((long)t * p.N + ring * 16 + cc) * H + slice * U + part * 4) = packed;
                }
            }
        }
        if (step + 1 < p.T) {
            const char* src = exr + (long)(step & 3) * slot_stride;
            __amdgpu_buffer_rsrc_t rs = __builtin_amdgcn_make_buffer_rsrc((void*)src, 0, TILE, 0x00020000);
#pragma unroll
            for (int kk = 0; kk < KQ; ++kk) {
                const int ks = wave + 4 * kk;
                if (EXACT || ks < NKS) hq[kk] = __builtin_amdgcn_raw_buffer_load_b128(rs, ks * 1024 + lo, 0, (int)0x80000010);
            }
        }
        const long long pc3 = (p.tune & 4) ? __builtin_readcyclecounter() : 0;
        x_phase(xbuf + ((step + 1) % 3) * TILE);
        if (p.tune & 4) {
            const long long now = __builtin_readcyclecounter();
            st_bar += pc2 - pc1; st_rec += pc3 - pc2; st_x += now - pc3;
            st_mf += pcm - pc2; st_gate += pcg - pcm; st_store += pc3 - pcg;
        }
    }
    if ((p.tune & 4) && lane == 0) {
        long long* st = (long long*)((char*)p.xcc_ws + (((size_t)p.n_rings * NSL * sizeof(int) + 64 + 7) & ~(size_t)7)) + ((long)ring * NSL + slice) * 16;
        st[0] = __builtin_readcyclecounter() - st_t0;
        st[1] = st_poll; st[2] = st_rounds; st[3] = st_first_ok; st[4] = st_x; st[5] = st_bar; st[6] = st_rec; st[7] = st_hist;
        st[8] = 0; st[9] = 0; st[10] = st_mf; st[11] = st_gate; st[12] = st_store;
        st[13] = (long long)__builtin_amdgcn_s_memrealtime() - st_r0;
    }
}

__device__ __forceinline__ void dma16_poll(const char* g, char* lds) {
    const unsigned l = (unsigned)__builtin_amdgcn_readfirstlane((int)(unsigned)(size_t)(__attribute__((address_space(3))) char*)lds);
    asm volatile("s_mov_b32 m0, %0\n\ts_nop 0\n\tglobal_load_lds_dwordx4 %1, off sc0 sc1" ::"s"(l), "v"(g) : "memory");
}
__device__ __forceinline__ void wait_vm(int n) {
    switch (n) {
        case 0: __builtin_amdgcn_s_waitcnt(0x0F70); break;
        case 1: __builtin_amdgcn_s_waitcnt(0x0F71); break;
        case 2: __builtin_amdgcn_s_waitcnt(0x0F72); break;
        case 3: __builtin_amdgcn_s_waitcnt(0x0F73); break;
        case 4: __builtin_amdgcn_s_waitcnt(0x0F74); break;
        case 5: __builtin_amdgcn_s_waitcnt(0x0F75); break;
        case 6: __builtin_amdgcn_s_waitcnt(0x0F76); break;
        case 7: __builtin_amdgcn_s_waitcnt(0x0F77); break;
        case 8: __builtin_amdgcn_s_waitcnt(0x0F78); break;
        case 9: __builtin_amdgcn_s_waitcnt(0x0F79); break;
        case 10: __builtin_amdgcn_s_waitcnt(0x0F7A); break;
        case 11: __builtin_amdgcn_s_waitcnt(0x0F7B); break;
        default: __builtin_amdgcn_s_waitcnt(0x0F7C); break;
    }
    asm volatile("" ::: "memory");
}

template <int NKS, int MT, bool STATS = false>
__global__ __launch_bounds__(256, 1) void lstm_layer_wgx2_kernel(LstmWgxArgs wp) {
    extern __shared__ __attribute__((aligned(16))) char smem[];
    const LstmFusedArgs& fp = wp.f;
    const LstmArgs& p = fp.a;
    constexpr int H = NKS * 32, U = 4 * MT, NSL = H / U, WPR = NSL / 4, KQ = (NKS + 3) / 4, TILE = NKS * 1024;
    constexpr bool EXACT = NKS % 4 == 0;
    static_assert(H % (4 * U) == 0, "four slices per workgroup");
    const int lane = threadIdx.x & 63;
    const int wave = __builtin_amdgcn_readfirstlane(threadIdx.x >> 6);
    const int xcd = blockIdx.x & 7;
    const int lwg = blockIdx.x >> 3;
    const int rl = lwg / WPR;
    const int n_pairs = (p.n_rings + 1) >> 1;
    const int pair = rl * 8 + ((p.tune & 32) ? ((xcd + (lwg - rl * WPR)) & 7) : xcd);
    const int slice = (lwg - rl * WPR) * 4 + wave;
    if (pair >= n_pairs) return;
    const int ring_of[2] = {pair, pair + n_pairs};
    const bool two = ring_of[1] < p.n_rings;

    char* hbuf = smem;
    char* xbuf = smem + 4 * TILE;
    char* stage = smem + 8 * TILE + wave * (16 * U * 2);

    half8_t whh[MT][NKS], wih[MT][NKS];
#pragma unroll
    for (int m = 0; m < MT; ++m)
#pragma unroll
        for (int ks = 0; ks < NKS; ++ks) {
            const long o = ((((long)slice * MT + m) * NKS + ks) * 64 + lane) * 8;
            whh[m][ks] = *(const half8_t*)(p.whh + o);
            wih[m][ks] = *(const half8_t*)(fp.wih + o);
        }
    const int c = lane & 15, q = lane >> 4;
    float4_t bias4[MT];
#pragma unroll
    for (int m = 0; m < MT; ++m)
#pragma unroll
        for (int i = 0; i < 4; ++i) bias4[m][i] = fp.bias[i * H + slice * U + q * MT + m];
    bool dead = false;
    const int dt = p.reverse ? -1 : 1;
    const int t0 = p.reverse ? p.T - 1 : 0;
    const long x_row = (long)p.N * H;
    const int lo = lane * 16;
    const long slot_stride = (long)wp.R * TILE;
    constexpr int PARTS = U / 4;
    const int ml = lane < 16 * PARTS ? lane : lane - 16 * PARTS;
    const int cc = ml / PARTS, part = ml - cc * PARTS;
    const int u0 = slice * U + part * 4;
    const int my_byte = (((u0 >> 5) * 64 + ((u0 >> 3) & 3) * 16 + cc) << 4) + (u0 & 7) * 2;
    int n_poll = 0, n_dma = 0;
#pragma unroll
    for (int kk = 0; kk < KQ; ++kk) {
        n_poll += (EXACT || wave + 4 * kk < NKS) ? 1 : 0;
        n_dma += (EXACT || (3 - wave) + 4 * kk < NKS) ? 1 : 0;
    }

    float cst[2][MT];
    float4_t xacc[2][MT];
    bool fast[2];
    const half_t* xptr[2];
    char* exr[2];
    int since[2] = {0, 0};
#pragma unroll
    for (int r = 0; r < 2; ++r) {
        const int ring = (r == 0 || two) ? ring_of[r] : ring_of[0];
        fast[r] = (r == 0 || two) ? ring_store_policy(p, ring, slice, NSL, lane) : false;
        xptr[r] = fp.x + ((long)(ring * 16 + c) * H + q * 8);
        exr[r] = wp.ex + (long)ring * TILE;
#pragma unroll
        for (int m = 0; m < MT; ++m) cst[r][m] = 0.f;
    }

    constexpr bool FASTPATH = NKS == 12 && MT == 3;
    const unsigned smem_a = lds_addr(smem);
    unsigned vx_off[2], vh_off[2], vp_off[KQ];
#pragma unroll
    for (int r = 0; r < 2; ++r) {
        const int ring = (r == 0 || two) ? ring_of[r] : ring_of[0];
        vx_off[r] = (unsigned)(((ring * 16 + c) * H + q * 8) * 2 + (3 - wave) * 64);
        vh_off[r] = (unsigned)(((ring * 16 + cc) * H + slice * U + part * 4) * 2);
    }
#pragma unroll
    for (int kk = 0; kk < KQ; ++kk) vp_off[kk] = (unsigned)(lo + (wave + 4 * kk) * 1024);
    const unsigned stage_a = lds_addr(stage);
    unsigned fast_u[2];
#pragma unroll
    for (int r = 0; r < 2; ++r)
        asm("s_cmp_lg_u64 %1, 0\n\ts_cselect_b32 %0, 1, 0" : "=s"(fast_u[r]) : "s"(__builtin_amdgcn_ballot_w64(fast[r])) : "scc");
    const long row_bytes = x_row * 2;
    const char* xrow2 = (const char*)fp.x + (long)(p.T > 2 ? t0 + 2 * dt : t0) * row_bytes;
    const char* xrow_any = (const char*)fp.x + (long)t0 * row_bytes;
    char* hrow = (char*)p.h + (long)t0 * row_bytes;

    auto x_phase = [&](const char* xb, float4_t (&xa)[MT]) {
#pragma unroll
        for (int m = 0; m < MT; ++m) xa[m] = bias4[m];
        half8_t b_cur = *(const half8_t*)(xb + lo), b_nxt = b_cur;
#pragma unroll
        for (int ks = 0; ks < NKS; ++ks) {
            if (ks + 1 < NKS) b_nxt = *(const half8_t*)(xb + (ks + 1) * 1024 + lo);
#pragma unroll
            for (int m = 0; m < MT; ++m) {
                if (m < MT - 1) mfma16_av(wih[m][ks], b_cur, xa[m]);
                else mfma16_vv(wih[m][ks], b_cur, xa[m]);
            }
            b_cur = b_nxt;
        }
        mfma_settle_v<MT>(xa);
    };
    auto x_dma = [&](const half_t* xp, char* xb, int tt, int slot) {
#pragma unroll
        for (int kk = 0; kk < KQ; ++kk) {
            const int ks = (3 - wave) + 4 * kk;
            if (EXACT || ks < NKS) dma16_wgx((const char*)(xp + (long)tt * x_row + ks * 32), xb + (slot * NKS + ks) * 1024);
        }
    };
    auto poll_dma = [&](const char* exbase, int slot, char* hb, unsigned mask) {
        const char* src = exbase + (long)slot * slot_stride + lo;
#pragma unroll
        for (int kk = 0; kk < KQ; ++kk) {
            const int ks = wave + 4 * kk;
            if ((EXACT || ks < NKS) && (mask & (1u << kk))) dma16_poll(src + ks * 1024, hb + ks * 1024);
        }
    };

#pragma unroll
    for (int r = 0; r < 2; ++r)
        if (r == 0 || two) {
            x_dma(xptr[r], xbuf + r * 2 * TILE, t0, 0);
            x_dma(xptr[r], xbuf + r * 2 * TILE, p.T > 1 ? t0 + dt : t0, 1);
        }
    if constexpr (NKS == 12 && MT == 3) {
#pragma unroll
        for (int r = 0; r < 2; ++r)
#pragma unroll
            for (int kk = 0; kk < KQ; ++kk)
                *(uint4_t*)(hbuf + r * 2 * TILE + (wave + 4 * kk) * 1024 + lo) = uint4_t{0u, 0u, 0u, 0u};
    }
    wait_vm(0);
    __syncthreads();
#pragma unroll
    for (int r = 0; r < 2; ++r)
        if (r == 0 || two) x_phase(xbuf + r * 2 * TILE, xacc[r]);

    long long st_poll = 0, st_bar = 0, st_slow = 0, st_sec[6] = {0, 0, 0, 0, 0, 0};
    const long long st_t0 = __builtin_readcyclecounter();
    const long long st_r0 = (p.tune & 4) ? (long long)__builtin_amdgcn_s_memrealtime() : 0;

    auto check_begin = [&](int rr, int st, uint4_t (&chk)[KQ]) {
        wait_vm(since[rr]);
        const char* hb = hbuf + (rr * 2 + (st & 1)) * TILE;
#pragma unroll
        for (int kk = 0; kk < KQ; ++kk) {
            const int ks = wave + 4 * kk;
            if (EXACT || ks < NKS) chk[kk] = *(const uint4_t*)(hb + ks * 1024 + lo);
        }
    };
    auto check_end = [&](int rr, int st, uint4_t (&chk)[KQ]) {
        char* hb = hbuf + (rr * 2 + (st & 1)) * TILE;
        unsigned spins = dead ? p.max_spins : 0u;
        while (true) {
            unsigned pend = 0;
#pragma unroll
            for (int kk = 0; kk < KQ; ++kk) {
                const int ks = wave + 4 * kk;
                if ((EXACT || ks < NKS) && __any(((chk[kk].x | chk[kk].y | chk[kk].z | chk[kk].w) & SENTINEL_MASK) != 0)) pend |= (1u << kk);
            }
            if (pend == 0) break;
            if (++spins > p.max_spins) {
                if (lane == 0 && !dead) atomicExch(p.err, 1);
                dead = true;
                break;
            }
            if (!(p.tune & 1)) __builtin_amdgcn_s_sleep(1);
            poll_dma(exr[rr], (st - 1) & 3, hb, pend);
            wait_vm(0);
#pragma unroll
            for (int kk = 0; kk < KQ; ++kk) {
                const int ks = wave + 4 * kk;
                if (EXACT || ks < NKS) chk[kk] = *(const uint4_t*)(hb + ks * 1024 + lo);
            }
        }
    };

    auto ring_step = [&](auto rc, auto two_c, int step, int t) {
        constexpr int r = decltype(rc)::value;
        constexpr bool TWO = decltype(two_c)::value;
        if constexpr (FASTPATH && TWO) {
            constexpr int o = r ^ 1;
            const int par = step & 1;
            const long long q0 = STATS ? __builtin_readcyclecounter() : 0;
            __syncthreads();
            const long long q1 = STATS ? __builtin_readcyclecounter() : 0;
            const int step_o = r == 0 ? step : step + 1;
            const bool chk_o = step_o >= 1 && step_o < p.T;
            const char* exo = exr[o] + (long)((step_o - 1) & 3) * slot_stride;
            const unsigned pm0 = (unsigned)__builtin_amdgcn_readfirstlane((int)(smem_a + (o * 2 + ((step_o & 1) ^ (chk_o ? 0 : 1))) * TILE + wave * 1024));
            const unsigned hbo = smem_a + (o * 2 + (step_o & 1)) * TILE + wave * 1024 + lo;
            const char* xsrc = (step + 2 < p.T) ? xrow2 : xrow_any;
            const unsigned xm0 = (unsigned)__builtin_amdgcn_readfirstlane((int)(smem_a + (4 + r * 2 + par) * TILE + (3 - wave) * 1024));
            unsigned long long bad;
            float hv[MT];
            const char* exs = exr[r] + (long)(step & 3) * slot_stride;
            const char* exa = exr[r] + (long)((step + 2) & 3) * slot_stride;
            ring_stream_paired<NKS, MT, KQ>(xacc[r], cst[r], hv, whh, wih, bias4, smem_a + (r * 2 + par) * TILE + lo,
                                            smem_a + (4 + r * 2 + (par ^ 1)) * TILE + lo, bad, pm0, exo, vp_off, xm0, xsrc, vx_off[r], hbo,
                                            stage_a + (unsigned)((c * U + q * MT) * 2), stage_a + (unsigned)((cc * U + part * 4) * 2),
                                            (unsigned)my_byte, vh_off[r], exs, exa, hrow, (unsigned)__builtin_amdgcn_readfirstlane((int)fast_u[r]));
            const long long q3 = STATS ? __builtin_readcyclecounter() : 0;
            if (__builtin_expect(chk_o && (bad != 0 || dead), 0)) {
                uint4_t chk[KQ];
#pragma unroll
                for (int kk = 0; kk < KQ; ++kk) chk[kk] = *(const uint4_t*)(hbuf + (o * 2 + (step_o & 1)) * TILE + (wave + 4 * kk) * 1024 + lo);
                check_end(o, step_o, chk);
                if constexpr (STATS) { st_poll += __builtin_readcyclecounter() - q3; ++st_slow; }
            }
            const long long q4 = STATS ? __builtin_readcyclecounter() : 0;
            if constexpr (STATS) {
                const long long q5 = __builtin_readcyclecounter();
                st_bar += q1 - q0; st_sec[2] += q3 - q1; st_sec[4] += q4 - q3; st_sec[3] += q5 - q4;
            }
            return;
        }
        char* hb_r = hbuf + (r * 2 + (step & 1)) * TILE;
        char* xb_r = xbuf + r * 2 * TILE;
        float4_t acc[MT];
// ... 68 lines not shown
        const long long pc7 = (p.tune & 4) ? __builtin_readcyclecounter() : 0;
        if (step + 1 < p.T) {
            poll_dma(exr[r], step & 3, hbuf + (r * 2 + ((step + 1) & 1)) * TILE, 0xFFu);
            since[r] = 0;
            since[r ^ 1] += n_poll;
        }
        if (p.tune & 4) {
            const long long pc8 = __builtin_readcyclecounter();
            st_sec[0] += pc3 - pc2; st_sec[1] += pc4 - pc3; st_sec[2] += pc5 - pc4; st_sec[3] += pc6 - pc5; st_sec[4] += pc7 - pc6; st_sec[5] += pc8 - pc7;
        }
    };

    const char* ex_slot[2][4];
#pragma unroll
    for (int r = 0; r < 2; ++r)
#pragma unroll
        for (int k = 0; k < 4; ++k) ex_slot[r][k] = exr[r] + (long)k * slot_stride;
    const unsigned lds_h = smem_a + lo;
    const unsigned lds_x = smem_a + 4 * TILE + lo;
    const unsigned lds_v = smem_a + wave * 1024 + lo;
    const unsigned m0_poll = (unsigned)__builtin_amdgcn_readfirstlane((int)(smem_a + wave * 1024));
    const unsigned m0_x = (unsigned)__builtin_amdgcn_readfirstlane((int)(smem_a + (3 - wave) * 1024));
    unsigned long long dead_m = 0;
    auto fast_step = [&](auto rc, auto phc, int step) {
        constexpr int r = decltype(rc)::value, ph = decltype(phc)::value, o = r ^ 1;
        constexpr int par = ph & 1, par_o = r == 0 ? par : par ^ 1;
        __syncthreads();
        unsigned long long bad;
        float hv[MT];
        ring_stream_unrolled<NKS, MT, KQ, (r * 2 + par) * TILE, (r * 2 + (par ^ 1)) * TILE, (o * 2 + par_o) * TILE, (o * 2 + par_o) * TILE,
                             (4 + r * 2 + par) * TILE>(
            xacc[r], cst[r], hv, whh, wih, bias4, lds_h, lds_x, bad, m0_poll, ex_slot[o][r == 0 ? (ph + 3) & 3 : ph], vp_off, m0_x, xrow2, vx_off[r],
            lds_v, stage_a + (unsigned)((c * U + q * MT) * 2), stage_a + (unsigned)((cc * U + part * 4) * 2), (unsigned)my_byte, vh_off[r],
            ex_slot[r][ph], ex_slot[r][(ph + 2) & 3], hrow, fast_u[r]);
        if (__builtin_expect((bad | dead_m) != 0, 0)) {
            const int step_o = r == 0 ? step : step + 1;
            uint4_t chk[KQ];
#pragma unroll
            for (int kk = 0; kk < KQ; ++kk) chk[kk] = *(const uint4_t*)(hbuf + (o * 2 + par_o) * TILE + (wave + 4 * kk) * 1024 + lo);
            check_end(o, step_o, chk);
            dead_m = __builtin_amdgcn_readfirstlane(dead ? 1 : 0) ? ~0ull : 0ull;
            if constexpr (STATS) ++st_slow;
        }
    };

    auto run = [&](auto two_c) {
        int t = t0;
        const long drow = dt * row_bytes;
        auto generic_steps = [&](int from, int to) {
            for (int step = from; step < to; ++step, t += dt) {
                ring_step(std::integral_constant<int, 0>{}, two_c, step, t);
                if constexpr (decltype(two_c)::value) ring_step(std::integral_constant<int, 1>{}, two_c, step, t);
                xrow2 += drow;
                hrow += drow;
            }
        };
        if constexpr (FASTPATH && decltype(two_c)::value) {
            int step = p.T < 4 ? p.T : 4;
            generic_steps(0, step);
            if (!(p.tune & 64) && fast_u[0] != 0 && fast_u[1] != 0) {
                for (; step + 4 <= p.T - 2; step += 4) {
                    fast_step(std::integral_constant<int, 0>{}, std::integral_constant<int, 0>{}, step);
                    fast_step(std::integral_constant<int, 1>{}, std::integral_constant<int, 0>{}, step);
                    xrow2 += drow; hrow += drow;
                    fast_step(std::integral_constant<int, 0>{}, std::integral_constant<int, 1>{}, step + 1);
                    fast_step(std::integral_constant<int, 1>{}, std::integral_constant<int, 1>{}, step + 1);
                    xrow2 += drow; hrow += drow;
                    fast_step(std::integral_constant<int, 0>{}, std::integral_constant<int, 2>{}, step + 2);
                    fast_step(std::integral_constant<int, 1>{}, std::integral_constant<int, 2>{}, step + 2);
                    xrow2 += drow; hrow += drow;
                    fast_step(std::integral_constant<int, 0>{}, std::integral_constant<int, 3>{}, step + 3);
                    fast_step(std::integral_constant<int, 1>{}, std::integral_constant<int, 3>{}, step + 3);
                    xrow2 += drow; hrow += drow;
                }
                t = t0 + step * dt;
            }
            generic_steps(step, p.T);
        } else {
            generic_steps(0, p.T);
        }
    };
    if (two) run(std::true_type{});
    else run(std::false_type{});
    wait_vm(0);
    if ((p.tune & 4) && lane == 0) {
        long long* st = (long long*)((char*)p.xcc_ws + (((size_t)p.n_rings * NSL * sizeof(int) + 64 + 7) & ~(size_t)7)) + ((long)ring_of[0] * NSL + slice) * 16;
        st[0] = __builtin_readcyclecounter() - st_t0;
        st[1] = st_poll; st[2] = st_slow; st[3] = 0; st[4] = 0; st[5] = st_bar; st[6] = 0; st[7] = st_sec[5];
        st[8] = st_sec[0]; st[9] = st_sec[1]; st[10] = st_sec[2]; st[11] = st_sec[3]; st[12] = st_sec[4];
        st[13] = (long long)__builtin_amdgcn_s_memrealtime() - st_r0;
    }
}

template <int NKS, int MT>
__global__ __launch_bounds__(64 * (NKS * 32 / (4 * MT)), 1) void lstm_layer_cta_kernel(LstmFusedArgs fp) {
    extern __shared__ __attribute__((aligned(16))) char smem[];
    const LstmArgs& p = fp.a;
    constexpr int H = NKS * 32, U = 4 * MT, NSL = H / U;
    static_assert(NSL >= NKS && NSL <= 16, "one workgroup per ring");
    const int lane = threadIdx.x & 63;
    const int slice = __builtin_amdgcn_readfirstlane(threadIdx.x >> 6);
    const int ring = blockIdx.x;
    char* hbuf = smem;
    char* xbuf = smem + 2 * NKS * 1024;

    half8_t whh[MT][NKS], wih[MT][NKS];
#pragma unroll
    for (int m = 0; m < MT; ++m)
#pragma unroll
        for (int ks = 0; ks < NKS; ++ks) {
            const long o = ((((long)slice * MT + m) * NKS + ks) * 64 + lane) * 8;
            whh[m][ks] = *(const half8_t*)(p.whh + o);
            wih[m][ks] = *(const half8_t*)(fp.wih + o);
        }
    const int c = lane & 15, q = lane >> 4;
    const int lo = lane * 16;
    float cst[MT];
    float4_t bias4[MT];
    int hoff[MT];
#pragma unroll
    for (int m = 0; m < MT; ++m) {
        cst[m] = 0.f;
        const int u = slice * U + q * MT + m;
#pragma unroll
        for (int i = 0; i < 4; ++i) bias4[m][i] = fp.bias[i * H + u];
        hoff[m] = (((u >> 5) * 64 + ((u >> 3) & 3) * 16 + c) * 16) + (u & 7) * 2;
    }
    int t = p.reverse ? p.T - 1 : 0;
    const int dt = p.reverse ? -1 : 1;
    const bool loader = slice < NKS;
    const half_t* xptr = fp.x + ((long)(ring * 16 + c) * H + slice * 32 + q * 8);
    half_t* hptr = p.h + ((long)(ring * 16 + c) * H + slice * 32 + q * 8);
    const long row = (long)p.N * H;

    uint4_t xq = {0, 0, 0, 0}, xr = {0, 0, 0, 0};
    float4_t xacc[MT];
    auto x_phase = [&](const char* xb) {
#pragma unroll
        for (int m = 0; m < MT; ++m) xacc[m] = bias4[m];
#pragma unroll
        for (int ks = 0; ks < NKS; ++ks) {
            const half8_t b = *(const half8_t*)(xb + ks * 1024 + lo);
#pragma unroll
            for (int m = 0; m < MT; ++m) xacc[m] = mfma16(wih[m][ks], b, xacc[m]);
        }
    };
    if (loader) {
        const int t1 = p.T > 1 ? t + dt : t, t2 = p.T > 2 ? t + 2 * dt : t, t3 = p.T > 3 ? t + 3 * dt : t;
        *(uint4_t*)(xbuf + slice * 1024 + lo) = *(const uint4_t*)(xptr + (long)t * row);
        *(uint4_t*)(xbuf + (NKS + slice) * 1024 + lo) = *(const uint4_t*)(xptr + (long)t1 * row);
        xq = *(const uint4_t*)(xptr + (long)t2 * row);
        xr = *(const uint4_t*)(xptr + (long)t3 * row);
    }
    __syncthreads();
    x_phase(xbuf);
    __syncthreads();

    for (int step = 0; step < p.T; ++step, t += dt) {
        const int par = step & 1;
        if (loader) {
            const int t4 = (step + 4 < p.T) ? t + 4 * dt : t;
            *(uint4_t*)(xbuf + (par * NKS + slice) * 1024 + lo) = xq;
            xq = xr;
            xr = *(const uint4_t*)(xptr + (long)t4 * row);
        }
        float4_t acc[MT];
#pragma unroll
// ... 191 lines not shown
                if (lane < 32) {
                    const int cc = lane >> 1, part = lane & 1;
                    const unsigned long long packed = *(const u64_alias_t*)((half_t*)stage + cc * U + part * 4);
                    unsigned long long* dst =
                        (unsigned long long*)(p.h + ((long)t * p.N + (ring * NB + nb) * 16 + cc) * H + slice * U + part * 4);
                    if constexpr (RX) {
                        const int u0 = slice * U + part * 4;
                        const int my_byte = (((nb * NKS + (u0 >> 5)) * 64 + ((u0 >> 3) & 3) * 16 + cc) << 4) + (u0 & 7) * 2;
                        __builtin_amdgcn_s_waitcnt(0x0F70);
                        unsigned long long* xd = (unsigned long long*)(exr + (long)(step & 3) * slot_stride + my_byte);
                        if (fast) *xd = packed;
                        else __hip_atomic_store(xd, packed, __ATOMIC_RELAXED, __HIP_MEMORY_SCOPE_AGENT);
                        if (step >= 2 && step + 2 < p.T) {
                            unsigned long long* ra = (unsigned long long*)(exr + (long)((step + 2) & 3) * slot_stride + my_byte);
                            if (fast) *ra = ~0ull;
                            else __hip_atomic_store(ra, ~0ull, __ATOMIC_RELAXED, __HIP_MEMORY_SCOPE_AGENT);
                        }
                        *dst = packed;
                    } else {
                        if (fast) *dst = packed;
                        else __hip_atomic_store(dst, packed, __ATOMIC_RELAXED, __HIP_MEMORY_SCOPE_AGENT);
                    }
                }
            }
            if (stats) { const long long c4 = __builtin_readcyclecounter(); st_poll += c1 - c0; st_bar += c2 - c1; st_mf += c3 - c2; st_gate += c4 - c3; }
        }
    }
    if (stats && lane == 0) {
        long long* st = (long long*)((char*)p.xcc_ws + (((size_t)p.n_rings * NSL * sizeof(int) + 64 + 7) & ~(size_t)7)) + ((long)ring * NSL + slice) * 16;
        st[0] = __builtin_readcyclecounter() - st_t0;
        st[1] = st_poll; st[2] = st_bar; st[3] = st_mf; st[4] = st_gate; st[5] = st_rounds;
        st[6] = (long long)__builtin_amdgcn_s_memrealtime() - st_r0; st[7] = st_wait;
    }
}

__global__ void fill_u16_kernel(uint16_t* dst, uint16_t v, size_t count) {
    size_t i = ((size_t)blockIdx.x * blockDim.x + threadIdx.x) * 8;
    const size_t stride = (size_t)gridDim.x * blockDim.x * 8;
    const unsigned vv = (unsigned)v | ((unsigned)v << 16);
    for (; i + 8 <= count; i += stride) *(uint4_t*)(dst + i) = uint4_t{vv, vv, vv, vv};
    if (i < count && i + 8 > count)
        for (size_t j = i; j < count; ++j) dst[j] = v;
}

}

static unsigned max_spins() { return (unsigned)bh::g_opt.lstm_max_spins; }

size_t bh_k_lstm_packed_bytes(int H) { return (size_t)4 * H * H * 2; }
size_t bh_k_lstm_ws_bytes(int N, int H) {
    const size_t waves = (size_t)((N + 15) / 16) * ((H + 7) / 8);
    return waves * sizeof(int) + 64 + waves * 16 * sizeof(long long) + 64;
}

int bh_k_fill_u16(void* dst, uint16_t value, size_t count, hipStream_t stream) {
    using namespace bh;
    BH_REQUIRE(((uintptr_t)dst & 15) == 0, "fill_u16: destination must be 16-byte aligned");
    size_t vecs = (count + 7) / 8;
    int blocks = (int)((vecs + 255) / 256);
    if (blocks > 4096) blocks = 4096;
    if (blocks < 1) blocks = 1;
    hipLaunchKernelGGL(fill_u16_kernel, dim3(blocks), dim3(256), 0, stream, (uint16_t*)dst, value, count);
    BH_CHECK_HIP(hipGetLastError());
    return 0;
}

bh_lstm_geometry bh_k_lstm_geometry(bh_lstm_family family, int H) {
    bh_lstm_geometry g;
    const int U = bh_k_lstm_wg_units(H);
    switch (family) {
        case BH_LSTM_WAVE:
        case BH_LSTM_FUSED: g.wgs_per_group = H / 16; g.rings_per_slot = 4; break;
        case BH_LSTM_STREAM: g.wgs_per_group = H / 64; break;
        case BH_LSTM_WGX2: g.rings_per_slot = 2; [[fallthrough]];
        case BH_LSTM_WGX: g.wgs_per_group = U ? H / (4 * U) : 0; break;
        case BH_LSTM_CTA: g.unlimited = true; break;
        case BH_LSTM_WIDE: g.ring_chunks = 32; g.wgs_per_group = H / 32; break;
        case BH_LSTM_Q8: break;
    }
    return g;
}

static int lstm_launch_prologue(const bh_lstm_geometry& g, int N, int R, int n_rings, int slots, int* xcc_ws, hipStream_t stream,
                                int* grid_out) {
    if (g.ring_chunks == 32) BH_REQUIRE(N % 32 == 0, "lstm: wide kernel needs the batch padded to a multiple of 32 (N=%d)", N);
    else BH_REQUIRE(N % 16 == 0, "lstm: batch must be padded to a multiple of 16 (N=%d)", N);
    BH_REQUIRE(n_rings > 0 && n_rings <= R, "lstm: n_rings=%d outside 1..%d", n_rings, R);
    const int grid = *grid_out = g.grid(n_rings);
    if (g.unlimited) return 0;
    const int cus = bh_cu_count();
    BH_REQUIRE(g.wgs_per_group > 0 && grid <= g.resident(cus), "lstm: %d workgroups must be co-resident but the device has %d CUs; split the batch", grid, cus);
    BH_REQUIRE(xcc_ws != nullptr, "lstm: missing XCD agreement workspace");
    BH_CHECK_HIP(hipMemsetAsync(xcc_ws, 0xFF, (size_t)n_rings * slots * sizeof(int), stream));
    return 0;
}

int bh_k_lstm_layer(const void* gates_in, const void* whh_packed, void* h_out, int T, int N, int H,
                    int reverse, int* err_flag, hipStream_t stream, int n_rings, int* xcc_ws, int force_slow) {
    using namespace bh;
    BH_REQUIRE(H % 32 == 0 && H >= 32 && H <= 512, "lstm: register-resident kernel needs H%%32==0, 32<=H<=512 (H=%d)", H);
    int grid = 0;
    if (int rc = lstm_launch_prologue(bh_k_lstm_geometry(BH_LSTM_WAVE, H), N, N / 16, n_rings, H / 16, xcc_ws, stream, &grid)) return rc;
    LstmArgs a{(const half_t*)gates_in, (const half_t*)whh_packed, (half_t*)h_out, T, N, H, n_rings,
               reverse, err_flag, max_spins(), xcc_ws, force_slow & 1, force_slow >> 8};
#define BH_LSTM_CASE(NKS) \
    case NKS: hipLaunchKernelGGL((lstm_layer_kernel<NKS, false>), dim3(grid), dim3(256), 0, stream, a); break;
    switch (H / 32) {
        BH_LSTM_CASE(1) BH_LSTM_CASE(2) BH_LSTM_CASE(3) BH_LSTM_CASE(4) BH_LSTM_CASE(5) BH_LSTM_CASE(6)
        BH_LSTM_CASE(7) BH_LSTM_CASE(8) BH_LSTM_CASE(9) BH_LSTM_CASE(10) BH_LSTM_CASE(11) BH_LSTM_CASE(12)
        BH_LSTM_CASE(13) BH_LSTM_CASE(14) BH_LSTM_CASE(15) BH_LSTM_CASE(16)
        default: BH_REQUIRE(false, "lstm: unsupported H=%d", H);
    }
#undef BH_LSTM_CASE
    BH_CHECK_HIP(hipGetLastError());
    return 0;
}

int bh_k_lstm_layer_stream(const void* gates_in, const void* whh_packed, void* h_out, int T, int N, int H,
                           int reverse, int* err_flag, hipStream_t stream, int n_rings, int* xcc_ws, int force_slow) {
    using namespace bh;
    BH_REQUIRE(H % 64 == 0 && H >= 64 && H <= 1024, "lstm: streaming kernel needs H%%64==0, 64<=H<=1024 (H=%d)", H);
    int grid = 0;
    if (int rc = lstm_launch_prologue(bh_k_lstm_geometry(BH_LSTM_STREAM, H), N, N / 16, n_rings, H / 16, xcc_ws, stream, &grid)) return rc;
    LstmArgs a{(const half_t*)gates_in, (const half_t*)whh_packed, (half_t*)h_out, T, N, H, n_rings,
               reverse, err_flag, max_spins(), xcc_ws, force_slow & 1, force_slow >> 8};
    switch (H / 32) {
        case 2: hipLaunchKernelGGL((lstm_layer_kernel<2, true>), dim3(grid), dim3(256), 0, stream, a); break;
        case 4: hipLaunchKernelGGL((lstm_layer_kernel<4, true>), dim3(grid), dim3(256), 0, stream, a); break;
        case 8: hipLaunchKernelGGL((lstm_layer_kernel<8, true>), dim3(grid), dim3(256), 0, stream, a); break;
        case 12: hipLaunchKernelGGL((lstm_layer_kernel<12, true>), dim3(grid), dim3(256), 0, stream, a); break;
        case 16: hipLaunchKernelGGL((lstm_layer_kernel<16, true>), dim3(grid), dim3(256), 0, stream, a); break;
        case 20: hipLaunchKernelGGL((lstm_layer_kernel<20, true>), dim3(grid), dim3(256), 0, stream, a); break;
        case 24: hipLaunchKernelGGL((lstm_layer_kernel<24, true>), dim3(grid), dim3(256), 0, stream, a); break;
        case 28: hipLaunchKernelGGL((lstm_layer_kernel<28, true>), dim3(grid), dim3(256), 0, stream, a); break;
        case 32: hipLaunchKernelGGL((lstm_layer_kernel<32, true>), dim3(grid), dim3(256), 0, stream, a); break;
        default: BH_REQUIRE(false, "lstm: unsupported H=%d for the streaming kernel", H);
    }
    BH_CHECK_HIP(hipGetLastError());
    return 0;
}

int bh_k_lstm_layer_fused(const void* x, const void* wih_packed, const float* bias, const void* whh_packed, void* h_out,
                          int T, int N, int H, int reverse, int* err_flag, hipStream_t stream, int n_rings, int* xcc_ws,
                          int force_slow) {
    using namespace bh;
    BH_REQUIRE(H % 32 == 0 && H >= 32 && H <= 512, "lstm: register-resident kernel needs H%%32==0, 32<=H<=512 (H=%d)", H);
    BH_REQUIRE(x != h_out, "lstm: fused layer cannot run in place");
    int grid = 0;
    if (int rc = lstm_launch_prologue(bh_k_lstm_geometry(BH_LSTM_FUSED, H), N, N / 16, n_rings, H / 16, xcc_ws, stream, &grid)) return rc;
    LstmFusedArgs a{(const half_t*)x, (const half_t*)wih_packed, bias,
                    LstmArgs{nullptr, (const half_t*)whh_packed, (half_t*)h_out, T, N, H, n_rings, reverse, err_flag, max_spins(),
                             xcc_ws, force_slow & 1, force_slow >> 8}};
    const size_t lds = (size_t)(H / 32) * 4096;
#define BH_LSTM_CASE(NKS)                                                                                        \
    case NKS:                                                                                                    \
        if (lds > 64 * 1024)                                                                                     \
            BH_CHECK_HIP(bh_max_lds((const void*)lstm_layer_fused_kernel<NKS>, (int)lds));            \
        hipLaunchKernelGGL(lstm_layer_fused_kernel<NKS>, dim3(grid), dim3(256), lds, stream, a);                 \
        break;
    switch (H / 32) {
        BH_LSTM_CASE(1) BH_LSTM_CASE(2) BH_LSTM_CASE(3) BH_LSTM_CASE(4) BH_LSTM_CASE(5) BH_LSTM_CASE(6)
        BH_LSTM_CASE(7) BH_LSTM_CASE(8) BH_LSTM_CASE(9) BH_LSTM_CASE(10) BH_LSTM_CASE(11) BH_LSTM_CASE(12)
        BH_LSTM_CASE(13) BH_LSTM_CASE(14) BH_LSTM_CASE(15) BH_LSTM_CASE(16)
        default: BH_REQUIRE(false, "lstm: unsupported H=%d", H);
    }
#undef BH_LSTM_CASE
    BH_CHECK_HIP(hipGetLastError());
    return 0;
}

int bh_k_lstm_wg_units(int H) {
    if (H % 32 != 0) return 0;
    const int nks = H / 32;
    if (H % 48 == 0 && nks <= 12) return 12;
    if (H % 64 == 0 && nks <= 8) return 16;
    return 0;
}

size_t bh_k_lstm_wgx_ex_bytes(int N, int H) { return (size_t)4 * (N / 16) * (H / 32) * 1024; }
int bh_k_lstm_layer_wgx(const void* x, const void* wih_packed, const float* bias, const void* whh_packed, void* h_out, void* ex,
                        int T, int N, int H, int R, int reverse, int* err_flag, hipStream_t stream, int n_rings, int* xcc_ws,
                        int force_slow, int arm) {
    using namespace bh;
    const int U = bh_k_lstm_wg_units(H);
    BH_REQUIRE(U != 0, "lstm: workgroup-shared kernel does not cover H=%d", H);
    BH_REQUIRE(x != h_out && ex != nullptr, "lstm: fused layer cannot run in place / missing exchange buffer");
    int grid = 0;
    if (int rc = lstm_launch_prologue(bh_k_lstm_geometry(BH_LSTM_WGX, H), N, R, n_rings, H / U, xcc_ws, stream, &grid)) return rc;
    const int nks = H / 32;
    if (arm) BH_CHECK_HIP(hipMemsetAsync(ex, 0xFF, (size_t)4 * R * nks * 1024, stream));
    LstmWgxArgs a{LstmFusedArgs{(const half_t*)x, (const half_t*)wih_packed, bias,
                                LstmArgs{nullptr, (const half_t*)whh_packed, (half_t*)h_out, T, N, H, n_rings, reverse, err_flag,
                                         max_spins(), xcc_ws, force_slow & 1, force_slow >> 8}},
                  (char*)ex, R};
    const size_t lds = (size_t)5 * nks * 1024 + 4 * 16 * U * 2;
#define BH_LSTM_WGX(NKS, MT)                                                                                     \
    if (nks == NKS && U == 4 * MT) {                                                                             \
        if (lds > 64 * 1024)                                                                                     \
            BH_CHECK_HIP(bh_max_lds((const void*)lstm_layer_wgx_kernel<NKS, MT>, (int)lds));            \
        hipLaunchKernelGGL((lstm_layer_wgx_kernel<NKS, MT>), dim3(grid), dim3(256), lds, stream, a);              \
    } else
    BH_LSTM_WGX(3, 3) BH_LSTM_WGX(6, 3) BH_LSTM_WGX(9, 3) BH_LSTM_WGX(12, 3)
    BH_LSTM_WGX(2, 4) BH_LSTM_WGX(4, 4) BH_LSTM_WGX(8, 4)
    { BH_REQUIRE(false, "lstm: workgroup-shared kernel has no instance for H=%d", H); }
#undef BH_LSTM_WGX
    BH_CHECK_HIP(hipGetLastError());
    return 0;
}

int bh_k_lstm_layer_wgx2(const void* x, const void* wih_packed, const float* bias, const void* whh_packed, void* h_out, void* ex,
                         int T, int N, int H, int R, int reverse, int* err_flag, hipStream_t stream, int n_rings, int* xcc_ws,
                         int force_slow, int arm) {
    using namespace bh;
    const int U = bh_k_lstm_wg_units(H);
    BH_REQUIRE(U != 0, "lstm: workgroup-shared kernel does not cover H=%d", H);
    BH_REQUIRE(x != h_out && ex != nullptr, "lstm: fused layer cannot run in place / missing exchange buffer");
    int grid = 0;
    if (int rc = lstm_launch_prologue(bh_k_lstm_geometry(BH_LSTM_WGX2, H), N, R, n_rings, H / U, xcc_ws, stream, &grid)) return rc;
    const int nks = H / 32;
    if (arm) BH_CHECK_HIP(hipMemsetAsync(ex, 0xFF, (size_t)4 * R * nks * 1024, stream));
    LstmWgxArgs a{LstmFusedArgs{(const half_t*)x, (const half_t*)wih_packed, bias,
                                LstmArgs{nullptr, (const half_t*)whh_packed, (half_t*)h_out, T, N, H, n_rings, reverse, err_flag,
                                         max_spins(), xcc_ws, force_slow & 1, force_slow >> 8}},
                  (char*)ex, R};
    const size_t lds = (size_t)8 * nks * 1024 + 4 * 16 * U * 2;
    if (nks == 12 && U == 12 && ((force_slow >> 8) & 4)) {
        BH_CHECK_HIP(bh_max_lds((const void*)lstm_layer_wgx2_kernel<12, 3, true>, (int)lds));
        hipLaunchKernelGGL((lstm_layer_wgx2_kernel<12, 3, true>), dim3(grid), dim3(256), lds, stream, a);
        BH_CHECK_HIP(hipGetLastError());
        return 0;
    }
#define BH_LSTM_WGX2(NKS, MT)                                                                                    \
    if (nks == NKS && U == 4 * MT) {                                                                             \
        if (lds > 64 * 1024)                                                                                     \
            BH_CHECK_HIP(bh_max_lds((const void*)lstm_layer_wgx2_kernel<NKS, MT>, (int)lds));            \
        hipLaunchKernelGGL((lstm_layer_wgx2_kernel<NKS, MT>), dim3(grid), dim3(256), lds, stream, a);             \
    } else
    BH_LSTM_WGX2(3, 3) BH_LSTM_WGX2(6, 3) BH_LSTM_WGX2(9, 3) BH_LSTM_WGX2(12, 3)
    BH_LSTM_WGX2(2, 4) BH_LSTM_WGX2(4, 4) BH_LSTM_WGX2(8, 4)
    { BH_REQUIRE(false, "lstm: workgroup-shared kernel has no instance for H=%d", H); }
#undef BH_LSTM_WGX2
    BH_CHECK_HIP(hipGetLastError());
    return 0;
}

int bh_k_lstm_cta_units(int H) {
    if (H == 96) return 12;
    if (H == 64 || H == 128) return 16;
    return 0;
}

int bh_k_lstm_layer_cta(const void* x, const void* wih_tiles, const float* bias, const void* whh_tiles, void* h_out, int T, int N,
                        int H, int reverse, hipStream_t stream, int n_rings) {
    using namespace bh;
    const int U = bh_k_lstm_cta_units(H);
    BH_REQUIRE(U != 0, "lstm: ring-in-a-workgroup kernel does not cover H=%d", H);
    BH_REQUIRE(x != h_out, "lstm: fused layer cannot run in place");
    int grid = 0;
    if (int rc = lstm_launch_prologue(bh_k_lstm_geometry(BH_LSTM_CTA, H), N, N / 16, n_rings, 0, nullptr, stream, &grid)) return rc;
    LstmFusedArgs a{(const half_t*)x, (const half_t*)wih_tiles, bias,
                    LstmArgs{nullptr, (const half_t*)whh_tiles, (half_t*)h_out, T, N, H, n_rings, reverse, nullptr, 0u, nullptr, 0, 0}};
    const int nks = H / 32, nsl = H / U;
    const size_t lds = (size_t)4 * nks * 1024;
    if (H == 96) hipLaunchKernelGGL((lstm_layer_cta_kernel<3, 3>), dim3(grid), dim3(64 * nsl), lds, stream, a);
    else if (H == 64) hipLaunchKernelGGL((lstm_layer_cta_kernel<2, 4>), dim3(grid), dim3(64 * nsl), lds, stream, a);
    else hipLaunchKernelGGL((lstm_layer_cta_kernel<4, 4>), dim3(grid), dim3(64 * nsl), lds, stream, a);
    BH_CHECK_HIP(hipGetLastError());
    return 0;
}

int bh_k_lstm_wide_ok(int H) { return H > 512 && H <= 1024 && H % 128 == 0; }

size_t bh_k_lstm_wide_ex_bytes(int N, int H) { return (size_t)4 * (N / 32) * 2 * (H / 32) * 1024; }

int bh_k_lstm_layer_wide(const void* gates_perm, const void* whh_tiles, void* h_out, int T, int N, int H, int reverse,
                         int* err_flag, hipStream_t stream, int n_rings, int* xcc_ws, int force_slow, void* ex, int R, int arm) {
    using namespace bh;
    BH_REQUIRE(bh_k_lstm_wide_ok(H), "lstm: wide kernel does not cover H=%d", H);
    int grid = 0;
    if (int rc = lstm_launch_prologue(bh_k_lstm_geometry(BH_LSTM_WIDE, H), N, N / 32, n_rings, H / 8, xcc_ws, stream, &grid)) return rc;
    LstmWideArgs a{(const half_t*)gates_perm,
                   LstmArgs{nullptr, (const half_t*)whh_tiles, (half_t*)h_out, T, N, H, n_rings, reverse, err_flag, max_spins(), xcc_ws,
                            force_slow & 1, force_slow >> 8},
                   (char*)ex, R};
    const int nks = H / 32;
    if (ex && arm) BH_CHECK_HIP(hipMemsetAsync(ex, 0xFF, (size_t)4 * R * 2 * nks * 1024, stream));
    const size_t lds = (size_t)2 * 2 * nks * 1024 + 4 * 16 * 8 * 2;
#define BH_LSTM_WIDE(NKS)                                                                                               \
    if (nks == NKS && ex) {                                                                                             \
        BH_CHECK_HIP(bh_max_lds((const void*)lstm_layer_wide_kernel<NKS, true>, (int)lds));                                                                    \
        hipLaunchKernelGGL((lstm_layer_wide_kernel<NKS, true>), dim3(grid), dim3(256), lds, stream, a);                  \
    } else if (nks == NKS) {                                                                                            \
        BH_CHECK_HIP(bh_max_lds((const void*)lstm_layer_wide_kernel<NKS, false>, (int)lds));                                                                    \
        hipLaunchKernelGGL((lstm_layer_wide_kernel<NKS, false>), dim3(grid), dim3(256), lds, stream, a);                 \
    } else
    if (nks == 32 && ex && ((force_slow >> 8) & 4)) {
        BH_CHECK_HIP(bh_max_lds((const void*)lstm_layer_wide_kernel<32, true, true>, (int)lds));
        hipLaunchKernelGGL((lstm_layer_wide_kernel<32, true, true>), dim3(grid), dim3(256), lds, stream, a);
    } else
    BH_LSTM_WIDE(20) BH_LSTM_WIDE(24) BH_LSTM_WIDE(28) BH_LSTM_WIDE(32)
    { BH_REQUIRE(false, "lstm: wide kernel has no instance for H=%d", H); }
#undef BH_LSTM_WIDE
    BH_CHECK_HIP(hipGetLastError());
    return 0;
}
```

### bonito_amd/csrc/options.cpp

```cpp
#include "options.h"

#include <string.h>

namespace bh {

Options g_opt;

#define BH_OPT(name) #name, &Options::name
static constexpr OptionRow OPTION_TABLE[] = {
    {BH_OPT(gemm_path), 0, Norm::keep, "linear GEMM kernel families: 0 auto, 1 = v1 only, 2 = no 256-tile kernel, 3 = no four-wave kernel, 5 = four-wave wherever legal"},
    {BH_OPT(gemm_tile16), 1, Norm::flag, "four-wave GEMM K-tile stream: 1 = 16x16x32 MFMAs, 0 = 32x32x16 (agree to fp16 rounding)"},
    {BH_OPT(gemm_order), 1, Norm::flag, "four-wave GEMM work order in an XCD: 1 = feature groups fastest, 0 = token blocks fastest (same bytes)"},
    {BH_OPT(gemm_gf), 0, Norm::keep, "four-wave GEMM feature tiles per block: 0 automatic, else rounded down to 1 / 2 / 4 / 8 / 16 / 32 (same bytes)"},
    {BH_OPT(gemm_stagger), 0, Norm::keep, "start-phase stagger of the persistent GEMM kernels, 0 = off (same bytes; measured without effect)"},
    {BH_OPT(attn_waves), 0, Norm::keep, "ring attention waves per workgroup: 0 automatic, 8, 12 (same results)"},
    {BH_OPT(attn_version), 2, Norm::one_or_two, "ring attention kernel: 2 = current, 1 = the first ring kernel"},
    {BH_OPT(attn_expt), 0, Norm::keep, "timing experiments of the ring attention kernel (bit mask): RESULTS ARE WRONG ON PURPOSE unless 0"},
    {BH_OPT(beam_fork), -1, Norm::keep, "posterior scan next to the beam kernel on a helper stream: -1 auto, 0 never, 1 always"},
    {BH_OPT(beam_select), 0, Norm::keep, "beam top-W selection: 0 histogram + boundary ranking, 1 radix search (same beams)"},
    {BH_OPT(beam_fuse), -1, Norm::keep, "forward / posterior scan as a second wave of the beam kernel: -1 auto (<= 256 states), 0 never, 1 always"},
    {BH_OPT(beam_cpw), 0, Norm::keep, "chunks per workgroup of the fused beam kernel at 256 states: 0 automatic, 1, 2, 4 (same bytes)"},
    {BH_OPT(decode_nt), 0, Norm::keep, "non-temporal score loads in the decode scans: 0 off"},
    {BH_OPT(viterbi_quad), 1, Norm::keep, "CRF Viterbi: 1 = four states per thread where the layout allows, 0 = the one-state kernel everywhere"},
    {BH_OPT(conv_ws), 1, Norm::keep, "weight-stationary kernel for the 384- / 96-channel 19-tap convolution: 1 on, 0 = generic implicit GEMM"},
    {BH_OPT(conv_fs), 1, Norm::keep, "feature-split instances of the implicit-GEMM convolution: 1 on, 0 = position-split"},
    {BH_OPT(conv_fuse), 1, Norm::keep, "conv1 -> conv2 -> conv3 as one kernel: 1 = 384-channel stacks, 2 = also 96-channel, 0 = three kernels"},
    {BH_OPT(conv_lds_kb), 64, Norm::positive_or_def, "KiB of LDS a workgroup of the implicit-GEMM convolution may take for its input span"},
    {BH_OPT(lstm_max_spins), 1000000, Norm::nonneg_or_def, "bound of the recurrent kernels' exchange spin loops (0: the first incomplete poll round is a timeout)"},
    {BH_OPT(lstm_q8_variant), 0, Norm::keep, "geometry of the 8-bit recurrent kernel, read at bh_encoder_create: 0, 1, 2"},
};
#undef BH_OPT

static constexpr bool defaults_agree() {
    constexpr Options o{};
    for (const OptionRow& r : OPTION_TABLE)
        if (o.*r.member != r.def) return false;
    return true;
}
static_assert(defaults_agree(), "options.h and OPTION_TABLE state different defaults");
static_assert(sizeof(OPTION_TABLE) / sizeof(OPTION_TABLE[0]) == sizeof(Options) / sizeof(int), "every member of Options has exactly one row");

const OptionRow* find_option(const char* name) {
    for (const OptionRow& r : OPTION_TABLE)
        if (!strcmp(name, r.name)) return &r;
    return nullptr;
}

}
```

### bonito_amd/csrc/options.h

```cpp
#pragma once

namespace bh {

struct Options {
    int gemm_path = 0;
    int gemm_tile16 = 1;
    int gemm_order = 1;
    int gemm_gf = 0;
    int gemm_stagger = 0;
    int attn_waves = 0;
    int attn_version = 2;
    int attn_expt = 0;
    int beam_fork = -1;
    int beam_select = 0;
    int beam_fuse = -1;
    int beam_cpw = 0;
    int decode_nt = 0;
    int viterbi_quad = 1;
    int conv_ws = 1;
    int conv_fs = 1;
    int conv_fuse = 1;
    int conv_lds_kb = 64;
    int lstm_max_spins = 1000000;
    int lstm_q8_variant = 0;
};
extern Options g_opt;

enum class Norm {
    keep,
    flag,
    one_or_two,
    positive_or_def,
    nonneg_or_def
};
struct OptionRow {
    const char* name;
    int Options::*member;
    int def;
    Norm norm;
    const char* what;
    int normalise(int v) const {
        switch (norm) {
            case Norm::flag: return v ? 1 : 0;
            case Norm::one_or_two: return v == 1 ? 1 : 2;
            case Norm::positive_or_def: return v > 0 ? v : def;
            case Norm::nonneg_or_def: return v >= 0 ? v : def;
            default: return v;
        }
    }
};
const OptionRow* find_option(const char* name);

}
```

### include/bonito_hip.h

```cpp
#ifndef BONITO_HIP_H
#define BONITO_HIP_H

#include <stddef.h>
#include <stdint.h>

#ifdef __cplusplus
extern "C" {
#endif

#define BH_ABI_VERSION 1

enum { BH_ACT_NONE = 0, BH_ACT_SWISH = 1, BH_ACT_TANH = 2, BH_ACT_RELU = 3 };

enum {
    BH_LAYER_CONV = 1,
    BH_LAYER_LSTM = 2,
    BH_LAYER_LINEAR_CRF = 3,
    BH_LAYER_CLAMP = 4,
    BH_LAYER_TRANSFORMER = 5,
    BH_LAYER_UPSAMPLE = 6,
    BH_LAYER_TCS_BLOCK = 7,
    BH_LAYER_CTC_DECODER = 8,
    BH_LAYER_DWCONV = 9,
    BH_LAYER_RESIDUAL_PROJ = 10,
    BH_LAYER_LINEAR = 11
};

typedef struct bh_layer {
    int32_t kind;
    int32_t in_size;
    int32_t out_size;
    int32_t winlen, stride, padding;
    int32_t activation;
    int32_t reverse;
    int32_t nhead, dim_ff, win_left, win_right;
    int32_t scale_factor;
    int32_t groups;
    int32_t add_residual;
    int32_t quantize;
    int32_t reserved_i[1];
    float scale;
    float clamp_lo, clamp_hi;
    float blank_score;
    float alpha;
    float eps;
    float reserved_f[2];
    const float* w0;
    const float* b0;
    const float* w1;
    const float* b1;
    const float* w2;
    const float* w3;
    const float* w4;
    const float* w5;
} bh_layer_t;

typedef struct bh_encoder bh_encoder_t;

const char* bh_last_error(void);
int bh_abi_version(void);
size_t bh_sizeof_layer(void);
int bh_device_count(void);

int bh_encoder_create(const bh_layer_t* layers, int n_layers, int device, int max_batch, int max_chunk,
                      bh_encoder_t** out);
void bh_encoder_destroy(bh_encoder_t* enc);
int bh_encoder_output_shape(const bh_encoder_t* enc, int L, int* T, int* C, int* stride);
int bh_encoder_forward(bh_encoder_t* enc, const void* signal, int N, int L, void* scores, void* stream);
int bh_encoder_describe(const bh_encoder_t* enc, char* buf, size_t bytes);
int bh_encoder_set_option(bh_encoder_t* enc, const char* name, int value);
int bh_encoder_debug_read(bh_encoder_t* enc, void* host, size_t bytes, size_t offset);
int bh_encoder_check(bh_encoder_t* enc, void* stream);
int bh_encoder_error_flag(const bh_encoder_t* enc);
long bh_encoder_last_ticket(const bh_encoder_t* enc);
int bh_encoder_error_flag_at(const bh_encoder_t* enc, long ticket);
int bh_encoder_ack(bh_encoder_t* enc, long ticket);

enum { BH_PROF_CONV = 0, BH_PROF_LSTM_GEMM = 1, BH_PROF_FILL = 2, BH_PROF_LSTM_REC = 3, BH_PROF_CRF_LINEAR = 4,
       BH_PROF_ATTENTION = 5 , BH_PROF_MLP = 6 ,
       BH_PROF_OTHER = 7, BH_PROF_MLP_FC1 = 8 ,
       BH_PROF_ATTENTION_CORE = 9 , BH_PROF_CLASSES = 10 };
int bh_encoder_profile(bh_encoder_t* enc, int enable);
int bh_encoder_profile_read(bh_encoder_t* enc, float* ms , int* spans );

size_t bh_crf_viterbi_workspace(int N, int T, int state_len);
int bh_crf_viterbi(const void* scores, int N, int T, int state_len, int layout_5s, float blank_score,
                   long stride_n, long stride_t, void* workspace, int8_t* moves, int8_t* path,
                   float* best, void* stream);

int bh_crf_reverse_complement(const void* in, void* out, int N, int T, int state_len, int layout_5s,
                              long stride_n, long stride_t, void* stream);
int bh_crf_logz(const void* scores, int N, int T, int state_len, float blank_score, void* workspace, double* logz,
                void* stream);

size_t bh_crf_seq_workspace(int N, int T, int Lmax, int state_len);
int bh_crf_seq_logz(const void* scores, int N, int T, int state_len, int layout_5s, float blank_score, long stride_n,
                    long stride_t, const void* targets, int Lmax, int target_bytes, const int32_t* target_lengths,
                    void* workspace, float* logz_out, void* stream);
int bh_crf_seq_viterbi(const void* scores, int N, int T, int state_len, int layout_5s, float blank_score, long stride_n,
                       long stride_t, const void* targets, int Lmax, int target_bytes, const int32_t* target_lengths,
                       void* workspace, int32_t* align_out, float* best_out, void* stream);
int bh_crf_seq_logz_free(const void* scores, int N, int T, int state_len, float blank_score, long stride_n, long stride_t,
                         const void* targets, int Lmax, int target_bytes, const int32_t* target_lengths, void* workspace,
                         float* logz_out, void* stream);
int bh_crf_logz_dense(const void* scores, int N, int T, int state_len, int layout_5s, float blank_score, long stride_n,
                      long stride_t, float* logz_out, void* stream);

size_t bh_sw_workspace(int n, int max_seq, int max_ref);
int bh_sw_align(const void* seqs, long seq_stride, const int32_t* seq_lengths, const void* refs, long ref_stride,
                const int32_t* ref_lengths, int n, int match, int mismatch, int gap_open, int gap_extend, void* workspace,
                size_t workspace_bytes, int32_t* result, uint32_t* ops, long ops_stride, int32_t* n_ops, void* stream);

int bh_signal_normalise(const int16_t* raw, const long* offsets, const float* cal_scale, const float* cal_offset, int n_reads,
                        int strategy, double quantile_a, double quantile_b, double shift_mult, double scale_mult,
                        double fixed_shift, double fixed_scale, int do_trim, double* shift, double* scale, int* weak, int* trim,
                        void* stream);
int bh_signal_chunks(const int16_t* raw, const long* offsets, const float* cal_scale, const float* cal_offset,
                     const double* shift, const double* scale, const int* weak, const int* chunk_read, const long* chunk_start,
                     const long* chunk_len, int n_chunks, int chunk_samples, void* out, void* stream);

int bh_lstm_q8_layer(const void* x, float bound, const float* w_ih, const float* w_hh, const float* bias, int T, int N, int H,
                     int reverse, int variant, void* h16_out, int8_t* hq_frag, int32_t* sums, void* stream);

int bh_set_option(const char* name, int value);

size_t bh_crf_posterior_viterbi_workspace(int N, int T, int state_len);
int bh_crf_posterior_viterbi(const void* scores, int N, int T, int state_len, float blank_score, void* workspace,
                             int8_t* moves, int8_t* path, void* stream);

size_t bh_beam_search_workspace(int N, int T, int state_len);
int bh_beam_search(const void* scores, int N, int T, int state_len, int beam_width, float beam_cut,
                   float blank_score, float q_scale, float q_offset, void* workspace, int8_t* sequence,
                   int8_t* qstring, int8_t* moves, float* qfloat, void* stream);

int bh_linear(const void* X, const void* W, const float* bias, void* out, int M, int N, int K, int ldx,
              int ldw, int ldo, int act, float scale, float clamp_lo, float clamp_hi, int gated,
              int row_div, long row_s_hi, long row_s_lo, int row_lim, void* stream);
int bh_linear_residual(const void* X, const void* W, const float* bias, void* out, int M, int N, int K, int ldx,
                       int ldw, int ldo, int act, float scale, float clamp_lo, float clamp_hi, int gated,
                       int row_div, long row_s_hi, long row_s_lo, int row_lim, const void* residual, int ldres,
                       float res_scale, void* stream);
int bh_linear_qkv_rotary(const void* X, const void* W, const float* bias, void* out, int M, int D, int K,
                         const float* cos_sin, int T, float qscale, void* stream);
int bh_linear_last_kernel(void);
int bh_conv1d_first(const void* signal, const float* w, const float* bias, void* out, int N, int Lin,
                    int Cout, int K, int stride, int pad, int act, float clamp_lo, float clamp_hi,
                    long os_n, long os_t, void* stream);
size_t bh_conv1d_packed_halves(int Cin, int Cout, int K);
int bh_conv1d_pack(const float* w, int Cin, int Cout, int K, uint16_t* packed);
int bh_conv1d(const void* in, const void* wpacked, const float* bias, void* out, int N, int Lin, int Cin,
              int Cout, int K, int stride, int pad, int act, float clamp_lo, float clamp_hi, long os_n,
              long os_t, void* stream);
int bh_ctc_greedy_decode(const float* logp, const long* offsets, int R, int classes, float qscale, float qbias,
                         int8_t* labels, int8_t* qual, int* path, int* count, void* stream);
// ... 30 lines not shown
```

Baseline: 342.8 million.

## Arm all LSTM ring-buffer flags with one memset per forward

Instead of issuing hipMemsetAsync fills of the XCD agreement slots and exchange buffers in front of every recurrent-kernel launch, each launch gets its own region of a larger workspace. All regions are set to 0xFF by a single fill at the start of the forward. This removes several small memset launches and their stream serialization between LSTM layers, at the cost of more device memory and more complex offset bookkeeping. It also adds optional per-workgroup timestamp instrumentation behind a compile flag, plus a query entry point for it.

```diff
diff --git a/bonito_amd/_lib.py b/bonito_amd/_lib.py
--- a/bonito_amd/_lib.py
+++ b/bonito_amd/_lib.py
@@ -93,6 +93,8 @@
     "bh_lstm_layer": (_i, [_vp, _vp, _vp, _i, _i, _i, _i, _vp, _vp, _i, _vp]),
     "bh_lstm_q8_layer": (_i, [_vp, _f, _vp, _vp, _vp, _i, _i, _i, _i, _i, _vp, _vp, _vp, _vp]),
     "bh_encoder_debug_read": (_i, [_vp, _vp, _sz, _sz]),
+    "bh_encoder_lstm_stamps": (_i, [_vp, _i, _vp, _sz]),
+    "bh_lstm_arm_bytes": (_sz, [_i, _i, _i, _i, _i, _vp]),
     "bh_encoder_set_option": (_i, [_vp, C.c_char_p, _i]),
 }
 
diff --git a/bonito_amd/csrc/abi.cpp b/bonito_amd/csrc/abi.cpp
--- a/bonito_amd/csrc/abi.cpp
+++ b/bonito_amd/csrc/abi.cpp
@@ -131,6 +131,9 @@
     return bh_k_dwconv(in, w, out, N, Lin, lout, C, K, stride, pad, (hipStream_t)stream);
 }
 extern "C" size_t bh_lstm_workspace(int N, int H) { return bh_k_lstm_ws_bytes(N, H); }
+extern "C" size_t bh_lstm_arm_bytes(int N, int H, int cus, int wide, int pairs, int* launches) {
+    return bh_k_lstm_arm_bytes(wide ? BH_LSTM_WIDE : BH_LSTM_WGX, N, H, cus, pairs, launches);
+}
 extern "C" int bh_lstm_layer(const void* gates_in, const void* whh_packed, void* h_out, int T, int N, int H,
                              int reverse, void* workspace, int* err_flag, int flags, void* stream) {
     BH_REQUIRE(gates_in && whh_packed && h_out && err_flag && workspace, "lstm_layer: null pointer");
diff --git a/bonito_amd/csrc/engine.cpp b/bonito_amd/csrc/engine.cpp
--- a/bonito_amd/csrc/engine.cpp
+++ b/bonito_amd/csrc/engine.cpp
@@ -128,6 +128,9 @@
     int lstm_prefill = 1;
     DevBuf q_act[2], q_ex;
     DevBuf ex16;
+    size_t arm_bytes = 0;
+    int arm_launches = 0;
+    int lstm_launches = 0;
     int lstm_pair = 1;
     int norm_fuse = 0;
     int lstm_exchange = 1;
@@ -533,7 +536,24 @@
             if (lstm_may_share(l.d)) exb = std::max(exb, bh_k_lstm_wgx_ex_bytes(Np, l.d.out_size));
             if (lstm_may_wide(l.d)) exb = std::max(exb, bh_k_lstm_wide_ex_bytes(Np, l.d.out_size));
         }
-        if (exb && e->ex16.alloc(exb + 256)) return -1;
+        size_t arm = 0;
+        int launches = 0;
+        for (const auto& l : e->layers) {
+            if (l.d.kind != BH_LAYER_LSTM) continue;
+            size_t b = 0;
+            int n = 0, n1 = 0;
+            if (lstm_may_share(l.d)) {
+                b = bh_k_lstm_arm_bytes(BH_LSTM_WGX, Np, l.d.out_size, e->n_cus, 0, &n);
+                b = std::max(b, bh_k_lstm_arm_bytes(BH_LSTM_WGX, Np, l.d.out_size, e->n_cus, 1, &n1));
+            }
+            if (lstm_may_wide(l.d)) b = std::max(b, bh_k_lstm_arm_bytes(BH_LSTM_WIDE, Np, l.d.out_size, e->n_cus, 0, &n1));
+            arm += b;
+            launches += std::max(n, n1);
+        }
+        e->arm_bytes = std::max(arm, exb ? exb + 256 : 0);
+        e->arm_launches = launches;
+        const size_t all = e->arm_bytes + (size_t)launches * BH_LSTM_STAMP_BYTES;
+        if (exb && (e->ex16.alloc(all) || hipMemset((char*)e->ex16.p + e->arm_bytes, 0, all - e->arm_bytes) != hipSuccess)) return -1;
     }
     if (e->act[0].alloc(ab + 256) || e->act[1].alloc(ab + 256) || e->gates.alloc(w.gate_bytes + 256) ||
         e->sig.alloc((size_t)Np * e->max_chunk * 2) || e->err.alloc(sizeof(int) * bh_encoder::ERR_SLOTS) ||
@@ -713,8 +733,18 @@
     hipStream_t st;
     void* scores;
     int n_act;
+    bool arm_once = false;
+    size_t arm_off = 0;
+    int lstm_launch = 0;
     void advance(void* dst) { cur = dst; which = (which + 1) % n_act; }
 };
+
+static size_t lstm_arm_bytes(const bh_encoder* e, const Layer& l, int Np, int* launches) {
+    const LstmPlan p = lstm_plan(e, l, Np);
+    if (launches) *launches = 0;
+    if (p.handoff != HANDOFF_RING || p.family == BH_LSTM_Q8) return 0;
+    return bh_k_lstm_arm_bytes(p.family, Np, l.d.out_size, e->n_cus, p.pairs, launches);
+}
 
 static int prefill_next(bh_encoder* e, const Cursor& c, size_t i, size_t rows) {
     if (e->n_act != 3 || !e->lstm_prefill || e->profiling) return 0;
@@ -860,6 +890,15 @@
     const int n_rings = p.n_rings, rev = d.reverse, slow = e->lstm_force_slow;
     int* ws = (int*)e->lstm_ws.p;
     const float* bias = (const float*)l.b0.p;
+    const bool ring_buf = p.handoff == HANDOFF_RING;
+    const bool armed = ring_buf && c.arm_once;
+    const int slots = p.family == BH_LSTM_WIDE ? H / 8 : bh_k_lstm_wg_units(H) ? H / bh_k_lstm_wg_units(H) : 0;
+    const auto arm_up = [](size_t b) { return (b + BH_LSTM_ARM_ALIGN - 1) / BH_LSTM_ARM_ALIGN * BH_LSTM_ARM_ALIGN; };
+    char* ex_base = (char*)e->ex16.p;
+    if (armed) {
+        ex_base += c.arm_off;
+        c.arm_off += arm_up(p.family == BH_LSTM_WIDE ? bh_k_lstm_wide_ex_bytes(Np, H) : bh_k_lstm_wgx_ex_bytes(Np, H));
+    }
     for (int r0 = 0; r0 < n_rings;) {
         const bool pair = p.pair_launch(n_rings - r0);
         const int nr = std::min(pair ? 2 * p.rings_per_launch : p.rings_per_launch, n_rings - r0);
@@ -867,17 +906,29 @@
         const char* x = (const char*)c.cur + col * H * 2;
         const char* g = (const char*)e->gates.p + col * 4 * H * 2;
         char* h = (char*)dst + col * H * 2;
-        char* ex = e->ex16.p ? (char*)e->ex16.p + (size_t)r0 * (p.geo.ring_chunks / 16) * (H / 32) * 1024 : nullptr;
+        char* ex = ex_base ? ex_base + (size_t)r0 * (p.geo.ring_chunks / 16) * (H / 32) * 1024 : nullptr;
+        int arm = r0 == 0 ? BH_LSTM_ARM_EX : BH_LSTM_ARM_SLOTS;
+        void* stamps = nullptr;
+        if (ring_buf) {
+            if (armed) {
+                arm = BH_LSTM_ARMED;
+                ws = (int*)((char*)e->ex16.p + c.arm_off);
+                c.arm_off += arm_up((size_t)nr * slots * sizeof(int));
+                BH_REQUIRE(c.arm_off <= e->arm_bytes, "encoder_forward: layer %zu leaves the armed workspace (%zu of %zu bytes)", i, c.arm_off, e->arm_bytes);
+            }
+            if (c.lstm_launch < e->arm_launches) stamps = (char*)e->ex16.p + e->arm_bytes + (size_t)c.lstm_launch * BH_LSTM_STAMP_BYTES;
+            ++c.lstm_launch;
+        }
         switch (pair ? BH_LSTM_WGX2 : p.family) {
             case BH_LSTM_WGX2:
-                rc = bh_k_lstm_layer_wgx2(x, l.w4.p, bias, l.w3.p, h, ex, len, Np, H, n_rings, rev, e->cur_err, st, nr, ws, slow, r0 == 0);
+                rc = bh_k_lstm_layer_wgx2(x, l.w4.p, bias, l.w3.p, h, ex, len, Np, H, n_rings, rev, e->cur_err, st, nr, ws, slow, arm, stamps);
                 break;
             case BH_LSTM_WGX:
-                rc = bh_k_lstm_layer_wgx(x, l.w4.p, bias, l.w3.p, h, ex, len, Np, H, n_rings, rev, e->cur_err, st, nr, ws, slow, r0 == 0);
+                rc = bh_k_lstm_layer_wgx(x, l.w4.p, bias, l.w3.p, h, ex, len, Np, H, n_rings, rev, e->cur_err, st, nr, ws, slow, arm);
                 break;
             case BH_LSTM_WIDE:
                 rc = bh_k_lstm_layer_wide(g, l.w3.p, h, len, Np, H, rev, e->cur_err, st, nr, ws, slow,
-                                          p.handoff == HANDOFF_RING ? ex : nullptr, n_rings, r0 == 0);
+                                          ring_buf ? ex : nullptr, n_rings, arm);
                 break;
             case BH_LSTM_CTA: rc = bh_k_lstm_layer_cta(x, l.w4.p, bias, l.w3.p, h, len, Np, H, rev, st, nr); break;
             case BH_LSTM_FUSED: rc = bh_k_lstm_layer_fused(x, l.w2.p, bias, l.w1.p, h, len, Np, H, rev, e->cur_err, st, nr, ws, slow); break;
@@ -1064,6 +1115,16 @@
     e->prefilled = nullptr;
     Cursor c;
     c.cur = e->sig.p; c.len = L; c.N = N; c.Np = Np; c.st = st; c.scores = scores; c.n_act = e->n_act;
+    if (bh::g_opt.lstm_arm_once && e->ex16.p && !((e->lstm_force_slow >> 8) & 4)) {
+        size_t bytes = 0;
+        for (const auto& l : e->layers)
+            if (l.d.kind == BH_LAYER_LSTM) bytes += lstm_arm_bytes(e, l, Np, nullptr);
+        if (bytes > 0 && bytes <= e->arm_bytes) {
+            ProfSpan span(e, st, BH_PROF_FILL);
+            BH_CHECK_HIP(hipMemsetAsync(e->ex16.p, 0xFF, bytes, st));
+            c.arm_once = true;
+        }
+    }
     for (size_t i = 0; i < e->layers.size(); ++i) {
         int rc = 0;
         switch (e->layers[i].d.kind) {
@@ -1081,6 +1142,7 @@
         }
         if (rc) return rc;
     }
+    e->lstm_launches = c.lstm_launch;
     BH_CHECK_HIP(hipMemcpyAsync(e->err_host + (e->cur_err - (int*)e->err.p), e->cur_err, sizeof(int), hipMemcpyDeviceToHost, st));
     return 0;
 }
@@ -1162,6 +1224,13 @@
     BH_REQUIRE(e && host && offset + bytes <= e->lstm_ws.bytes, "encoder_debug_read: out of range");
     BH_CHECK_HIP(hipMemcpy(host, (char*)e->lstm_ws.p + offset, bytes, hipMemcpyDeviceToHost));
     return 0;
+}
+extern "C" int bh_encoder_lstm_stamps(bh_encoder_t* e, int launch, void* host, size_t bytes) {
+    BH_REQUIRE(e && host, "encoder_lstm_stamps: null argument");
+    BH_REQUIRE(launch >= 0 && launch < e->arm_launches && bytes <= BH_LSTM_STAMP_BYTES, "encoder_lstm_stamps: launch %d / %zu bytes out of range", launch, bytes);
+    BH_CHECK_HIP(hipDeviceSynchronize());
+    BH_CHECK_HIP(hipMemcpy(host, (char*)e->ex16.p + e->arm_bytes + (size_t)launch * BH_LSTM_STAMP_BYTES, bytes, hipMemcpyDeviceToHost));
+    return e->lstm_launches;
 }
 extern "C" int bh_encoder_set_option(bh_encoder_t* e, const char* name, int value) {
     BH_REQUIRE(e && name, "encoder_set_option: null argument");
diff --git a/bonito_amd/csrc/kernels.h b/bonito_amd/csrc/kernels.h
--- a/bonito_amd/csrc/kernels.h
+++ b/bonito_amd/csrc/kernels.h
@@ -126,9 +126,16 @@
                        void* hq_out, void* h16_out, void* ex, int T, int N, int H, int R, int n_rings, int reverse, int* err_flag,
                        hipStream_t stream, int* xcc_ws, int flags, int variant, int* dbg, unsigned max_spins);
 size_t bh_k_lstm_wgx_ex_bytes(int N, int H);
+enum { BH_LSTM_ARM_SLOTS = 0,
+       BH_LSTM_ARM_EX = 1,
+       BH_LSTM_ARMED = 2 };
+constexpr size_t BH_LSTM_ARM_ALIGN = 256;
+size_t bh_k_lstm_arm_bytes(bh_lstm_family family, int N, int H, int cus, int pairs, int* launches);
+constexpr int BH_LSTM_STAMP_WORDS = 16, BH_LSTM_STAMP_WGS = 512;
+constexpr size_t BH_LSTM_STAMP_BYTES = (size_t)BH_LSTM_STAMP_WGS * BH_LSTM_STAMP_WORDS * 8;
 int bh_k_lstm_layer_wgx(const void* x, const void* wih_tiles, const float* bias, const void* whh_tiles, void* h_out, void* ex, int T,
                         int N, int H, int R, int reverse, int* err_flag, hipStream_t stream, int n_rings, int* xcc_ws, int force_slow,
                         int arm);
 int bh_k_lstm_layer_wgx2(const void* x, const void* wih_tiles, const float* bias, const void* whh_tiles, void* h_out, void* ex, int T,
                         int N, int H, int R, int reverse, int* err_flag, hipStream_t stream, int n_rings, int* xcc_ws, int force_slow,
-                        int arm);
+                        int arm, void* stamps = nullptr);
diff --git a/bonito_amd/csrc/lstm.hip b/bonito_amd/csrc/lstm.hip
--- a/bonito_amd/csrc/lstm.hip
+++ b/bonito_amd/csrc/lstm.hip
@@ -1,4 +1,5 @@
 #include <string.h>
+#include <algorithm>
 #include <type_traits>
 
 #include "common.h"
@@ -413,7 +414,21 @@
     LstmFusedArgs f;
     char* ex;
     int R;
+#ifdef BH_LSTM_STATS
+    long long* stamps;
+#endif
 };
+
+enum LstmStamp { STAMP_ENTRY, STAMP_HANDSHAKE, STAMP_WEIGHTS, STAMP_LOOP, STAMP_LOOP_END, STAMP_EXIT, STAMP_COUNT };
+#ifdef BH_LSTM_STATS
+#define BH_LSTM_STAMP(i)                                                           \
+    do {                                                                           \
+        stamp_c[i] = (long long)__builtin_amdgcn_s_memtime();                      \
+        stamp_r[i] = (long long)__builtin_amdgcn_s_memrealtime();                  \
+    } while (0)
+#else
+#define BH_LSTM_STAMP(i) do { } while (0)
+#endif
 
 template <int IMM, bool POLL>
 __device__ __forceinline__ void dma16_s(const char* sbase, unsigned voff, unsigned lds_a) {
@@ -702,6 +717,10 @@
     constexpr int H = NKS * 32, U = 4 * MT, NSL = H / U, WPR = NSL / 4, KQ = (NKS + 3) / 4, TILE = NKS * 1024;
     constexpr bool EXACT = NKS % 4 == 0;
     static_assert(H % (4 * U) == 0, "four slices per workgroup");
+#ifdef BH_LSTM_STATS
+    long long stamp_c[STAMP_COUNT], stamp_r[STAMP_COUNT];
+#endif
+    BH_LSTM_STAMP(STAMP_ENTRY);
     const int lane = threadIdx.x & 63;
     const int wave = __builtin_amdgcn_readfirstlane(threadIdx.x >> 6);
     const int xcd = blockIdx.x & 7;
@@ -766,6 +785,11 @@
 #pragma unroll
         for (int m = 0; m < MT; ++m) cst[r][m] = 0.f;
     }
+    BH_LSTM_STAMP(STAMP_HANDSHAKE);
+#ifdef BH_LSTM_STATS
+    wait_vm(0);
+    BH_LSTM_STAMP(STAMP_WEIGHTS);
+#endif
 
     constexpr bool FASTPATH = NKS == 12 && MT == 3;
     const unsigned smem_a = lds_addr(smem);
@@ -838,6 +862,7 @@
 #pragma unroll
     for (int r = 0; r < 2; ++r)
         if (r == 0 || two) x_phase(xbuf + r * 2 * TILE, xacc[r]);
+    BH_LSTM_STAMP(STAMP_LOOP);
 
     long long st_poll = 0, st_bar = 0, st_slow = 0, st_sec[6] = {0, 0, 0, 0, 0, 0};
     const long long st_t0 = __builtin_readcyclecounter();
@@ -1072,7 +1097,17 @@
     };
     if (two) run(std::true_type{});
     else run(std::false_type{});
+    BH_LSTM_STAMP(STAMP_LOOP_END);
     wait_vm(0);
+#ifdef BH_LSTM_STATS
+    BH_LSTM_STAMP(STAMP_EXIT);
+    if (wp.stamps && wave == 0 && lane == 0) {
+        long long* sw = wp.stamps + (long)blockIdx.x * BH_LSTM_STAMP_WORDS;
+#pragma unroll
+        for (int i = 0; i < STAMP_COUNT; ++i) { sw[i] = stamp_c[i]; sw[8 + i] = stamp_r[i]; }
+        sw[6] = pair; sw[7] = xcc_id(); sw[14] = p.T; sw[15] = 1;
+    }
+#endif
     if ((p.tune & 4) && lane == 0) {
         long long* st = (long long*)((char*)p.xcc_ws + (((size_t)p.n_rings * NSL * sizeof(int) + 64 + 7) & ~(size_t)7)) + ((long)ring_of[0] * NSL + slice) * 16;
         st[0] = __builtin_readcyclecounter() - st_t0;
@@ -1430,7 +1465,7 @@
 }
 
 static int lstm_launch_prologue(const bh_lstm_geometry& g, int N, int R, int n_rings, int slots, int* xcc_ws, hipStream_t stream,
-                                int* grid_out) {
+                                int* grid_out, bool armed = false) {
     if (g.ring_chunks == 32) BH_REQUIRE(N % 32 == 0, "lstm: wide kernel needs the batch padded to a multiple of 32 (N=%d)", N);
     else BH_REQUIRE(N % 16 == 0, "lstm: batch must be padded to a multiple of 16 (N=%d)", N);
     BH_REQUIRE(n_rings > 0 && n_rings <= R, "lstm: n_rings=%d outside 1..%d", n_rings, R);
@@ -1439,7 +1474,7 @@
     const int cus = bh_cu_count();
     BH_REQUIRE(g.wgs_per_group > 0 && grid <= g.resident(cus), "lstm: %d workgroups must be co-resident but the device has %d CUs; split the batch", grid, cus);
     BH_REQUIRE(xcc_ws != nullptr, "lstm: missing XCD agreement workspace");
-    BH_CHECK_HIP(hipMemsetAsync(xcc_ws, 0xFF, (size_t)n_rings * slots * sizeof(int), stream));
+    if (!armed) BH_CHECK_HIP(hipMemsetAsync(xcc_ws, 0xFF, (size_t)n_rings * slots * sizeof(int), stream));
     return 0;
 }
 
@@ -1526,6 +1561,26 @@
 }
 
 size_t bh_k_lstm_wgx_ex_bytes(int N, int H) { return (size_t)4 * (N / 16) * (H / 32) * 1024; }
+
+size_t bh_k_lstm_arm_bytes(bh_lstm_family family, int N, int H, int cus, int pairs, int* launches) {
+    if (launches) *launches = 0;
+    if (family != BH_LSTM_WGX && family != BH_LSTM_WIDE) return 0;
+    const bh_lstm_geometry g = bh_k_lstm_geometry(family, H);
+    const int slots = family == BH_LSTM_WIDE ? H / 8 : H / (bh_k_lstm_wg_units(H) ? bh_k_lstm_wg_units(H) : 16);
+    const int n_rings = N / g.ring_chunks, per = g.rings_per_launch(cus);
+    if (n_rings <= 0 || per <= 0) return 0;
+    auto up = [](size_t b) { return (b + BH_LSTM_ARM_ALIGN - 1) / BH_LSTM_ARM_ALIGN * BH_LSTM_ARM_ALIGN; };
+    size_t bytes = up(family == BH_LSTM_WIDE ? bh_k_lstm_wide_ex_bytes(N, H) : bh_k_lstm_wgx_ex_bytes(N, H));
+    int n = 0;
+    for (int r0 = 0; r0 < n_rings; ++n) {
+        const bool pair = family == BH_LSTM_WGX && pairs && n_rings - r0 > per;
+        const int nr = std::min(pair ? 2 * per : per, n_rings - r0);
+        bytes += up((size_t)nr * slots * sizeof(int));
+        r0 += nr;
+    }
+    if (launches) *launches = n;
+    return bytes;
+}
 int bh_k_lstm_layer_wgx(const void* x, const void* wih_packed, const float* bias, const void* whh_packed, void* h_out, void* ex,
                         int T, int N, int H, int R, int reverse, int* err_flag, hipStream_t stream, int n_rings, int* xcc_ws,
                         int force_slow, int arm) {
@@ -1534,9 +1589,9 @@
     BH_REQUIRE(U != 0, "lstm: workgroup-shared kernel does not cover H=%d", H);
     BH_REQUIRE(x != h_out && ex != nullptr, "lstm: fused layer cannot run in place / missing exchange buffer");
     int grid = 0;
-    if (int rc = lstm_launch_prologue(bh_k_lstm_geometry(BH_LSTM_WGX, H), N, R, n_rings, H / U, xcc_ws, stream, &grid)) return rc;
+    if (int rc = lstm_launch_prologue(bh_k_lstm_geometry(BH_LSTM_WGX, H), N, R, n_rings, H / U, xcc_ws, stream, &grid, arm == BH_LSTM_ARMED)) return rc;
     const int nks = H / 32;
-    if (arm) BH_CHECK_HIP(hipMemsetAsync(ex, 0xFF, (size_t)4 * R * nks * 1024, stream));
+    if (arm == BH_LSTM_ARM_EX) BH_CHECK_HIP(hipMemsetAsync(ex, 0xFF, (size_t)4 * R * nks * 1024, stream));
     LstmWgxArgs a{LstmFusedArgs{(const half_t*)x, (const half_t*)wih_packed, bias,
                                 LstmArgs{nullptr, (const half_t*)whh_packed, (half_t*)h_out, T, N, H, n_rings, reverse, err_flag,
                                          max_spins(), xcc_ws, force_slow & 1, force_slow >> 8}},
@@ -1558,19 +1613,25 @@
 
 int bh_k_lstm_layer_wgx2(const void* x, const void* wih_packed, const float* bias, const void* whh_packed, void* h_out, void* ex,
                          int T, int N, int H, int R, int reverse, int* err_flag, hipStream_t stream, int n_rings, int* xcc_ws,
-                         int force_slow, int arm) {
+                         int force_slow, int arm, void* stamps) {
     using namespace bh;
     const int U = bh_k_lstm_wg_units(H);
     BH_REQUIRE(U != 0, "lstm: workgroup-shared kernel does not cover H=%d", H);
     BH_REQUIRE(x != h_out && ex != nullptr, "lstm: fused layer cannot run in place / missing exchange buffer");
     int grid = 0;
-    if (int rc = lstm_launch_prologue(bh_k_lstm_geometry(BH_LSTM_WGX2, H), N, R, n_rings, H / U, xcc_ws, stream, &grid)) return rc;
+    if (int rc = lstm_launch_prologue(bh_k_lstm_geometry(BH_LSTM_WGX2, H), N, R, n_rings, H / U, xcc_ws, stream, &grid, arm == BH_LSTM_ARMED)) return rc;
     const int nks = H / 32;
-    if (arm) BH_CHECK_HIP(hipMemsetAsync(ex, 0xFF, (size_t)4 * R * nks * 1024, stream));
+    if (arm == BH_LSTM_ARM_EX) BH_CHECK_HIP(hipMemsetAsync(ex, 0xFF, (size_t)4 * R * nks * 1024, stream));
     LstmWgxArgs a{LstmFusedArgs{(const half_t*)x, (const half_t*)wih_packed, bias,
                                 LstmArgs{nullptr, (const half_t*)whh_packed, (half_t*)h_out, T, N, H, n_rings, reverse, err_flag,
                                          max_spins(), xcc_ws, force_slow & 1, force_slow >> 8}},
                   (char*)ex, R};
+#ifdef BH_LSTM_STATS
+    a.stamps = (long long*)stamps;
+    BH_REQUIRE(!stamps || grid <= BH_LSTM_STAMP_WGS, "lstm: %d workgroups, the stamp block holds %d", grid, BH_LSTM_STAMP_WGS);
+#else
+    (void)stamps;
+#endif
     const size_t lds = (size_t)8 * nks * 1024 + 4 * 16 * U * 2;
     if (nks == 12 && U == 12 && ((force_slow >> 8) & 4)) {
         BH_CHECK_HIP(bh_max_lds((const void*)lstm_layer_wgx2_kernel<12, 3, true>, (int)lds));
@@ -1626,13 +1687,13 @@
     using namespace bh;
     BH_REQUIRE(bh_k_lstm_wide_ok(H), "lstm: wide kernel does not cover H=%d", H);
     int grid = 0;
-    if (int rc = lstm_launch_prologue(bh_k_lstm_geometry(BH_LSTM_WIDE, H), N, N / 32, n_rings, H / 8, xcc_ws, stream, &grid)) return rc;
+    if (int rc = lstm_launch_prologue(bh_k_lstm_geometry(BH_LSTM_WIDE, H), N, N / 32, n_rings, H / 8, xcc_ws, stream, &grid, arm == BH_LSTM_ARMED)) return rc;
     LstmWideArgs a{(const half_t*)gates_perm,
                    LstmArgs{nullptr, (const half_t*)whh_tiles, (half_t*)h_out, T, N, H, n_rings, reverse, err_flag, max_spins(), xcc_ws,
                             force_slow & 1, force_slow >> 8},
                    (char*)ex, R};
     const int nks = H / 32;
-    if (ex && arm) BH_CHECK_HIP(hipMemsetAsync(ex, 0xFF, (size_t)4 * R * 2 * nks * 1024, stream));
+    if (ex && arm == BH_LSTM_ARM_EX) BH_CHECK_HIP(hipMemsetAsync(ex, 0xFF, (size_t)4 * R * 2 * nks * 1024, stream));
     const size_t lds = (size_t)2 * 2 * nks * 1024 + 4 * 16 * 8 * 2;
 #define BH_LSTM_WIDE(NKS)                                                                                               \
     if (nks == NKS && ex) {                                                                                             \
diff --git a/bonito_amd/csrc/options.cpp b/bonito_amd/csrc/options.cpp
--- a/bonito_amd/csrc/options.cpp
+++ b/bonito_amd/csrc/options.cpp
@@ -28,6 +28,7 @@
     {BH_OPT(conv_lds_kb), 64, Norm::positive_or_def, "KiB of LDS a workgroup of the implicit-GEMM convolution may take for its input span"},
     {BH_OPT(lstm_max_spins), 1000000, Norm::nonneg_or_def, "bound of the recurrent kernels' exchange spin loops (0: the first incomplete poll round is a timeout)"},
     {BH_OPT(lstm_q8_variant), 0, Norm::keep, "geometry of the 8-bit recurrent kernel, read at bh_encoder_create: 0, 1, 2"},
+    {BH_OPT(lstm_arm_once), 1, Norm::flag, "fp16 ring-buffer recurrent kernels: 1 = one fill at the top of a forward arms every launch, 0 = fills in front of every launch (same bytes)"},
 };
 #undef BH_OPT
 
diff --git a/bonito_amd/csrc/options.h b/bonito_amd/csrc/options.h
--- a/bonito_amd/csrc/options.h
+++ b/bonito_amd/csrc/options.h
@@ -23,6 +23,7 @@
     int conv_lds_kb = 64;
     int lstm_max_spins = 1000000;
     int lstm_q8_variant = 0;
+    int lstm_arm_once = 1;
 };
 extern Options g_opt;
 
diff --git a/include/bonito_hip.h b/include/bonito_hip.h
--- a/include/bonito_hip.h
+++ b/include/bonito_hip.h
@@ -70,6 +70,8 @@
 int bh_encoder_describe(const bh_encoder_t* enc, char* buf, size_t bytes);
 int bh_encoder_set_option(bh_encoder_t* enc, const char* name, int value);
 int bh_encoder_debug_read(bh_encoder_t* enc, void* host, size_t bytes, size_t offset);
+int bh_encoder_lstm_stamps(bh_encoder_t* enc, int launch, void* host, size_t bytes);
+size_t bh_lstm_arm_bytes(int N, int H, int cus, int wide, int pairs, int* launches);
 int bh_encoder_check(bh_encoder_t* enc, void* stream);
 int bh_encoder_error_flag(const bh_encoder_t* enc);
 long bh_encoder_last_ticket(const bh_encoder_t* enc);
```

Measured after the change: 343.4 million (median of 6 runs). About the same (+0.2%).
